# a-lemus96/fs-nerf

Measured on AMD Instinct MI355X. Metric: rendered rays/sec (64+128 samples/ray, 8x256 MLP), higher is better.
Workload: dtype fp16x3

## Files before the change

### fs-nerf_amd/core/models.py

```python
import warnings
from typing import Optional, Sequence, Tuple

import torch
from torch import Tensor, nn
from torch.autograd.function import once_differentiable

from .. import _lib as L
from .. import ops


def _freqs(n_freqs: int, log_space: bool) -> Tensor:
    if log_space:
        return 2.0 ** torch.linspace(0.0, n_freqs - 1, n_freqs)
    return torch.linspace(2.0 ** 0.0, 2.0 ** (n_freqs - 1), n_freqs)


class PositionalEncoder(nn.Module):
    def __init__(self, d_input: int, n_freqs: int, log_space: bool = False):
        super().__init__()
        self.d_input, self.n_freqs, self.log_space = d_input, n_freqs, log_space
        self.d_output = d_input * (1 + 2 * n_freqs)
        self.freqs = [float(f) for f in _freqs(n_freqs, log_space)] if n_freqs > 0 else []

    def forward(self, x: Tensor, mask: Optional[Tensor] = None) -> Tensor:
# ... 155 lines not shown
        self.pos_mask, self.dir_mask = pos_mask, dir_mask

    def train_prec(self) -> int:
        tp = self.train_precision or self.precision
        if tp == "fp16x2":
            tp = "fp16x3"
        return self.PRECISIONS[tp]

    @staticmethod
    def fp16_family(prec: int) -> bool:
        return prec in (L.FSN_PREC_FP16X3, L.FSN_PREC_FP16, L.FSN_PREC_FP16X2)

    @property
    def fp16_mode(self) -> bool:
        return self.fp16_family(self.PRECISIONS[self.precision])

    def _bwd_stage_state(self, dev, which: str = ""):
        st = getattr(self, "_bwd_stage" + which)
        if st is None or st[0].device != dev:
            n = self.n_layers + 2
            st = (torch.ones(n, dtype=torch.float32, device=dev), torch.zeros(n, dtype=torch.int32, device=dev))
            setattr(self, "_bwd_stage" + which, st)
            setattr(self, "_bwd_calibrated" + which, False)
        return st

    def _fold_input_status(self, word: Tensor, dev) -> None:
        w = self._input_word
        if w is None or w.device != dev:
            w = self._input_word = torch.zeros(1, dtype=torch.int32, device=dev)
        w.bitwise_or_(word)
        self._input_calls += 1
        if self.range_check and self._input_calls % self.range_check_every == 0:
            bits = int(w.item())
            if bits:
                w.zero_()
            if bits & L.FSN_STATUS_GRAD_RANGE:
                self.grad_overflow_looks += 1
            if bits & (L.FSN_STATUS_FP16_RANGE | L.FSN_STATUS_FP16_SMALL):
                self.fall_back("input-gradient calls (a flagged call's gradients were written as zeros)", bits, scaled=False)

    def _step_flags(self, dev):
        flags, loose = {}, False
        for p in self.parameters():
            f = getattr(p, "_fsn_step_flag", None)
            if f is None or f.device != dev:
                loose = True
            else:
                flags[id(f)] = f
        out = list(flags.values())
        if loose or not out:
            out.append(ops.step_flag(dev))
        return out

    def _train_status(self, dev) -> Tensor:
        w = self._train_word
        if w is None or w.device != dev:
            w = self._train_word = torch.zeros(2, dtype=torch.int32, device=dev)
        return w

    def fold_status(self, word: Tensor, dev, slot: int) -> None:
        for f in self._step_flags(dev):
            f.bitwise_or_(word)
        self._train_status(dev)[slot:slot + 1].bitwise_or_(word)

    def _read_train_status(self, dev) -> Tuple[int, int]:
        w = self._train_status(dev)
        from ..shard import max_bits_over_ranks
        local, samp = (int(v) for v in w.tolist())
        if local & L.FSN_STATUS_GRAD_RANGE:
            self.grad_overflow_looks += 1
        env = L.FSN_STATUS_FP16_RANGE | L.FSN_STATUS_FP16_SMALL
        bits = max_bits_over_ranks(local & env, dev)
        sbits = max_bits_over_ranks(samp & env, dev)
        if local or samp or bits or sbits:
            w.zero_()
        return bits & env, sbits & env

    def fall_back(self, what: str, bits: int = L.FSN_STATUS_FP16_RANGE, probe=None, earlier_invalid: bool = False,
                  scaled: bool = True) -> None:
        self.range_events += 1
        if scaled and self.infer_prec() == L.FSN_PREC_FP16X3U and self._recalibrate(bits, probe):
            if earlier_invalid:
                warnings.warn(f"fs-nerf HIP path: {what}: the per-layer activation scales did not fit the data "
                              f"({ops.describe_flags(bits)}); re-calibrated", RuntimeWarning, stacklevel=3)
            return
        new = self.FALLBACK.get(self.precision, "bf16x3")
        warnings.warn(f"fs-nerf HIP path: {what}: hidden activations left the fp16 range envelope of precision "
                      f"'{self.precision}' ({ops.describe_flags(bits)}); re-running / continuing in '{new}'",
                      RuntimeWarning, stacklevel=3)
        self.precision = new
        if self.train_precision in self.FALLBACK:
            self.train_precision = None

    def _tensors(self):
        mods = list(self.layers) + [self.sigma, self.connection, self.branch, self.rgb]
        return [m.weight for m in mods], [m.bias for m in mods]

    ACT_TARGET_EXP = 10
    PROBE_MAX = 16384

    def infer_prec(self) -> int:
        if self.precision == "fp16x3" and self.act_scaling:
            return L.FSN_PREC_FP16X3U
        return self.PRECISIONS[self.precision]

    def _param_key(self):
        ws, bs = self._tensors()
        return tuple((t.data_ptr(), t._version) for t in ws + bs)

    def load_state_dict(self, *args, **kwargs):
        out = super().load_state_dict(*args, **kwargs)
        self._act_exps = None
        self._forget_target_moves()
        return out

    def _forget_target_moves(self) -> None:
        self.act_target_exp -= self._target_moved_by
        self._target_moved_by = self._calib_moves = 0

    def _default_probe(self, dev):
        g = torch.Generator(device="cpu").manual_seed(0)
        x = (torch.rand(4096, 3, generator=g) * 4.0 - 2.0).to(dev)
        d = torch.nn.functional.normalize(torch.randn(4096, 3, generator=g), dim=-1).to(dev)
        return x, d

    @torch.no_grad()
    def calibrate(self, probe=None, keep_if_close: bool = False) -> list:
        import math
        ws, bs = self._tensors()
        dev = ws[0].device
        if callable(probe):
            probe = probe()
        x, d = probe if probe is not None else self._default_probe(dev)
        x, d = x.reshape(-1, 3).to(dev, torch.float32), d.reshape(-1, 3).to(dev, torch.float32)
        if x.shape[0] == 0:
            x, d = self._default_probe(dev)
        if x.shape[0] > self.PROBE_MAX:
            idx = torch.linspace(0, x.shape[0] - 1, self.PROBE_MAX, device=dev).long()
            x, d = x[idx], d[idx]
        desc = ops.make_desc(self.n_layers, self.d_hidden, self.skip, self.pos_encoder.freqs, self.dir_encoder.freqs)
        if self._calib_blob is None or self._calib_blob.blob.device != dev:
            self._calib_blob = ops.PackedMLP(desc, L.FSN_PREC_BF16X3, dev)
        self._calib_blob.pack(ws, bs)
        maxima = ops.mlp_layer_maxima(self._calib_blob, x.contiguous(), d.contiguous(), self._mask(self.pos_mask, dev),
                                      self._mask(self.dir_mask, dev))
        D, n = self.d_hidden, self.n_layers
        mods = list(self.layers) + [self.connection, self.branch]
        wmax = []
        for g, m in enumerate(mods):
            w = m.weight.detach().abs()
            na = 0 if g == 0 else D
            wmax.append(w[:, :na].amax() if na else w.new_zeros(()))
            wmax.append(w[:, na:].amax() if w.shape[1] > na else w.new_zeros(()))
        host = torch.cat([maxima, torch.stack(wmax).to(torch.float32)]).cpu().tolist()
        amax, wmx = host[:n + 2], host[n + 2:]
        T = int(self.act_target_exp)
        old = self._act_exps
        exps = []
        for g, v in enumerate(amax):
            if not math.isfinite(v):
                raise RuntimeError(f"NeRF.calibrate: layer {g} produced non-finite activations on the probe batch")
            if v <= 0.0:
                e = old[g] if old is not None else 0
            else:
                e = T - math.ceil(math.log2(v))
                if keep_if_close and old is not None and 2.0 ** (T - 3) <= v * 2.0 ** old[g] <= 2.0 ** (T + 1):
                    e = old[g]
            exps.append(max(-60, min(60, e)))
        for g in range(n + 2):
            prev = 0 if g == 0 else (exps[n - 1] if g == n else (exps[n] if g == n + 1 else exps[g - 1]))
            for wm, sh in ((wmx[2 * g], exps[g] - prev), (wmx[2 * g + 1], exps[g])):
                if wm > 0.0 and math.isfinite(wm):
                    over = math.ceil(math.log2(wm)) + sh - 15
                    if over > 0:
                        exps[g] -= over
        self._act_exps = exps
        self._calib_key = self._param_key()
        self._needs_calibration = False
        self.calibrations += 1
        return exps

    def _recalibrate(self, bits: int, probe) -> bool:
        if self._act_exps is not None and self._calib_key == self._param_key():
            if self._calib_moves >= 3 or bits == (L.FSN_STATUS_FP16_RANGE | L.FSN_STATUS_FP16_SMALL):
                return False
            self._calib_moves += 1
            move = -4 if bits & L.FSN_STATUS_FP16_RANGE else 3
            self.act_target_exp += move
            self._target_moved_by += move
            if not 2 <= self.act_target_exp <= 14:
                return False
        else:
            self._forget_target_moves()
        try:
            self.calibrate(probe)
        except RuntimeError:
            return False
        return True

    def _weights_below_envelope(self) -> bool:
        mods = list(self.layers) + [self.connection, self.branch]
        with torch.no_grad():
            m = torch.stack([mod.weight.detach().abs().amax() for mod in mods])
            return bool(((m > 0) & (m < 2.0 ** -20)).any())

    def _guard_weights(self, what: str, training: bool = False) -> None:
        if not training and self.infer_prec() == L.FSN_PREC_FP16X3U:
            return
        if self.range_check and self.weight_check and self.fp16_mode and self._weights_below_envelope():
            self.fall_back(what + " (a layer's largest weight is below 2^-20)", L.FSN_STATUS_FP16_SMALL, scaled=False)

    def packed(self, probe=None) -> ops.PackedMLP:
        ws, bs = self._tensors()
        scaled = self.infer_prec() == L.FSN_PREC_FP16X3U
        if scaled and (self._act_exps is None or self._needs_calibration):
            self.calibrate(probe, keep_if_close=self._act_exps is not None)
        exps = tuple(self._act_exps) if scaled else None
        key = (self.precision, ws[0].device, exps) + self._param_key()
        if self._packed is None or key != self._packed_key:
            if self._pack_calls % max(1, int(self.range_check_every)) == 0:
                self._guard_weights("NeRF.packed")
                scaled = self.infer_prec() == L.FSN_PREC_FP16X3U
                exps = tuple(self._act_exps) if scaled else None
                key = (self.precision, key[1], exps) + key[3:]
            self._pack_calls += 1
            desc = ops.make_desc(self.n_layers, self.d_hidden, self.skip, self.pos_encoder.freqs,
                                 self.dir_encoder.freqs)
            prec = self.infer_prec()
            if self._packed is None or self._packed.prec != prec or self._packed.blob.device != ws[0].device:
                self._packed = ops.PackedMLP(desc, prec, ws[0].device)
            self._packed.pack(ws, bs, exps)
            self._packed_key = key
        return self._packed

    def packed_single(self, precision: str) -> ops.PackedMLP:
        if precision not in self.SINGLE_PASS:
            raise ValueError(f"single-pass precision: one of {self.SINGLE_PASS}, not {precision!r}")
        ws, bs = self._tensors()
        key = (ws[0].device,) + self._param_key()
        ent = self._packed_single.get(precision)
        if ent is None or ent[0] != key:
            pm = None if ent is None else ent[1]
            if pm is None or pm.blob.device != ws[0].device:
                desc = ops.make_desc(self.n_layers, self.d_hidden, self.skip, self.pos_encoder.freqs, self.dir_encoder.freqs)
                pm = ops.PackedMLP(desc, self.PRECISIONS[precision], ws[0].device)
            pm.pack(ws, bs)
            self._packed_single[precision] = (key, pm)
        return self._packed_single[precision][1]

    def packed_cull(self) -> ops.PackedMLP:
        if self.cull_precision != "bf16":
            raise ValueError("NeRF.cull_precision: None or 'bf16'")
        return self.packed_single(self.cull_precision)

    def occ_eval_fn(self, render_step_size: float, precision: str = "fp16") -> "OccEvalFn":
        return OccEvalFn(self, render_step_size, precision)

    def _autocast_mode(self) -> Optional[str]:
        ap = self.autocast_precision
        if ap is None:
            return None
        if ap not in self.SINGLE_PASS:
            raise ValueError(f"NeRF.autocast_precision: None or one of {self.SINGLE_PASS}, not {ap!r}")
        return ap if not torch.is_grad_enabled() and torch.is_autocast_enabled("cuda") else None

    def _leave_fp16_autocast(self, what: str, bits: int) -> str:
        self.autocast_precision = "bf16"
        return _warn_single_pass(self, what, bits)

    def _mask(self, m: Optional[Tensor], dev) -> Optional[Tensor]:
        return None if m is None else m.to(dev, torch.float32)

    def forward_rays(self, rays_o: Tensor, rays_d: Tensor, ray_indices: Tensor, t_starts: Tensor, t_ends: Tensor,
                     full: bool = True) -> Tensor:
        if full and self._differentiable(rays_o, rays_d):
            ws, bs = self._tensors()
            return _NerfTrainFn.apply(self, (ray_indices, t_starts, t_ends), rays_o, rays_d, *ws, *bs)
        dev = rays_o.device
        args = (rays_o, rays_d, ray_indices, t_starts, t_ends, full, self._mask(self.pos_mask, dev), self._mask(self.dir_mask, dev))

        def probe():
            n = ray_indices.numel()
            idx = torch.linspace(0, max(n - 1, 0), min(n, self.PROBE_MAX), device=dev).long()
            ri = ray_indices[idx].long()
            d = rays_d[ri]
            return rays_o[ri] + d * (t_starts[idx] + t_ends[idx])[:, None] / 2.0, d

        return guarded_launch([self], dev, "NeRF.forward_rays", probe, lambda: ops.mlp_fwd_rays(self.packed(probe), *args))

    def _differentiable(self, *inputs: Optional[Tensor]) -> bool:
        if not torch.is_grad_enabled():
            return False
        if self.training and any(p.requires_grad for p in self.parameters()):
            return True
        return any(t is not None and t.requires_grad for t in inputs)

    def density_gradient(self, x: Tensor) -> Tuple[Tensor, Tensor]:
        xg = x.detach().reshape(-1, 3).to(torch.float32).contiguous().requires_grad_(True)
        dirs = torch.tensor([0.0, 0.0, 1.0], device=xg.device).expand(xg.shape[0], 3).contiguous()
        ws, bs = self._tensors()
        with torch.enable_grad():
            out = _NerfTrainFn.apply(self, None, xg, dirs, *[t.detach() for t in ws + bs])
            cot = torch.zeros_like(out)
            cot[:, 3] = 1.0
            (grad,) = torch.autograd.grad(out, xg, cot)
        return out[:, 3].detach(), grad

    def forward(self, x: Tensor, dirs: Optional[Tensor] = None) -> Tensor:
        if self._differentiable(x, dirs):
            if dirs is None:
                if not self._differentiable():
                    return self._forward_inference(x, dirs)
                raise NotImplementedError(
                    "NeRF.forward(x) with gradients: the density-only pass has no backward (the reference runs it "
                    "under torch.no_grad(), rendering.py:58-64); call it under torch.no_grad() (density_gradient(x) gives "
                    "sigma and its gradient with respect to x)")
            ws, bs = self._tensors()
            return _NerfTrainFn.apply(self, None, x, dirs, *ws, *bs)
        return self._forward_inference(x, dirs)

    def _forward_inference(self, x: Tensor, dirs: Optional[Tensor]) -> Tensor:
        dev = x.device
        mode = self._autocast_mode()
        if mode is not None:
            return single_pass_launch(self, mode, dev, "NeRF.forward (autocast_precision)", self._leave_fp16_autocast,
                                      lambda pm: ops.mlp_fwd(pm, x, dirs, self._mask(self.pos_mask, dev),
                                                             self._mask(self.dir_mask, dev)))

# ... 93 lines not shown
```

### fs-nerf_amd/csrc/host_pack.cpp

```cpp
#include <cstdarg>
#include <cstdio>

#include "mlp_pack.hpp"

static thread_local char g_err[512] = "";
static void set_error(const char* fmt, ...) {
  va_list ap;
  va_start(ap, fmt);
  vsnprintf(g_err, sizeof(g_err), fmt, ap);
  va_end(ap);
}

extern "C" int fsn_version(void) { return 200; }
extern "C" const char* fsn_last_error(void) { return g_err; }

extern "C" int64_t fsn_mlp_blob_bytes(const fsn_mlp_desc* desc, int prec) {
  if (!desc) { set_error("fsn_mlp_blob_bytes: null desc"); return FSN_E_INVALID; }
  fsn::NetGeom G;
  const char* why;
  const int rc = fsn::build_geom(*desc, prec, G, &why);
  if (rc != FSN_OK) { set_error("fsn_mlp_blob_bytes: %s", why); return rc; }
  return G.total_bytes;
}

extern "C" int fsn_mlp_pack_host(const fsn_mlp_desc* desc, int prec, const float* const* weights,
                                 const float* const* biases, void* blob_host) {
  if (!blob_host) { set_error("fsn_mlp_pack_host: null blob"); return FSN_E_INVALID; }
  const char* why;
  const int rc = fsn::pack_blob_host(desc, prec, weights, biases, blob_host, &why);
  if (rc != FSN_OK) set_error("fsn_mlp_pack_host: %s", why);
  return rc;
}

extern "C" int fsn_mlp_pack_scaled_host(const fsn_mlp_desc* desc, int prec, const float* const* weights,
                                        const float* const* biases, const int32_t* layer_exps, void* blob_host) {
  if (!blob_host) { set_error("fsn_mlp_pack_scaled_host: null blob"); return FSN_E_INVALID; }
  const char* why;
  const int rc = fsn::pack_blob_host(desc, prec, weights, biases, blob_host, &why, layer_exps);
  if (rc != FSN_OK) set_error("fsn_mlp_pack_scaled_host: %s", why);
  return rc;
}
```

### fs-nerf_amd/csrc/mlp.hip

```cpp
#include "common.hpp"
#define FSN_X3_PF1
#define FSN_BF16X3_ONEACC 1
#include "mlp_dev.hpp"
#include "mlp_layout.hpp"
#include "mlp_pack.hpp"

#include <cstring>
#include <vector>

namespace fsn {

__global__ void k_pack_stream(PackArgs a, char* __restrict__ blob, int64_t n_pieces) {
  const int64_t piece = (int64_t)blockIdx.x * blockDim.x + threadIdx.x;
  if (piece >= n_pieces) return;
  uint16_t o[8];
  pack_piece(a, piece, o);
  uint4 v;
  v.x = o[0] | ((uint32_t)o[1] << 16);
  v.y = o[2] | ((uint32_t)o[3] << 16);
  v.z = o[4] | ((uint32_t)o[5] << 16);
  v.w = o[6] | ((uint32_t)o[7] << 16);
  *reinterpret_cast<uint4*>(blob + a.G.stream_off + piece * 16) = v;
}

__global__ void k_pack_aux(PackArgs a, char* __restrict__ blob) {
  const int i = blockIdx.x * blockDim.x + threadIdx.x;
  if (i < 64) {
    uint32_t hw[64];
    header_words(a, hw);
    uint32_t w = 0;
#pragma unroll
    for (int k = 0; k < 64; ++k) w = (k == i) ? hw[k] : w;
    reinterpret_cast<uint32_t*>(blob)[i] = w;
  }
  if (i < a.G.aux_floats) reinterpret_cast<float*>(blob + a.G.aux_off)[i] = aux_value(a, i);
}

static int fill_pack_args(const fsn_mlp_desc* d, int prec, const float* const* W, const float* const* b,
                          PackArgs& a, const int32_t* exps = nullptr) {
  const char* why;
  const int rc = fill_pack_args_raw(d, prec, W, b, a, &why, exps);
  FSN_REQUIRE(rc == FSN_OK, rc, "mlp_pack: %s", why);
  return FSN_OK;
}

struct MlpFwdArgs {
  NetParams net;
  const float* x;
  const float* dirs;
  const float* pos_mask;
  const float* dir_mask;
  int64_t n;
  float* out;
  const float *rays_o, *rays_d, *t0, *t1;
  const int64_t* ri;
  int32_t full;
};

template <int NT, int PREC, bool FULL>
__global__ __launch_bounds__(kThreads) void k_mlp_fwd(MlpFwdArgs a) {
  constexpr int NG = groups_per_wave<NT, PREC>(), TILE = 128 * NG;
  __shared__ __attribute__((aligned(1024))) char smem[kRingBytes + (kAuxCapFloats + 96) * 4 + TILE * 6 * 4];
  float* aux_lds = reinterpret_cast<float*>(smem + kRingBytes);
  float* in_lds = aux_lds + kAuxCapFloats + 96;
  NetDev net;
  load_net(a.net, a.pos_mask, a.dir_mask, aux_lds, net);
  __syncthreads();
  constexpr bool full = FULL;
  const int64_t ntiles = (a.n + TILE - 1) / TILE;
  WStream st;
  const char* sbase = a.net.blob + a.net.stream_off;
  st.init(smem, nullptr, 0, 0, sbase, (uint32_t)(full ? a.net.nph_full : a.net.nph_density), 1);
  const int wave = threadIdx.x >> 6, lane = threadIdx.x & 63;
  ARing ring;
  prime_ring<PREC, NT>(st, ring);
  for (int64_t tile = blockIdx.x; tile < ntiles; tile += gridDim.x) {
    if (lane < 16 * NG) {
      const int64_t s = tile * TILE + wave * (16 * NG) + lane;
      const int64_t sc = s < a.n ? s : a.n - 1;
      float* q = in_lds + (wave * (16 * NG) + lane) * 6;
      if (a.ri) {
        ray_sample(a.rays_o, a.rays_d, a.ri, a.t0, a.t1, sc, q, full);
      } else {
        q[0] = a.x[3 * sc]; q[1] = a.x[3 * sc + 1]; q[2] = a.x[3 * sc + 2];
        if (full) { q[3] = a.dirs[3 * sc]; q[4] = a.dirs[3 * sc + 1]; q[5] = a.dirs[3 * sc + 2]; }
      }
    }
    __builtin_amdgcn_wave_barrier();
    const int64_t s0 = tile * TILE + tile_slot<NG>(wave, lane, 0);
    TileSrc src[NG];
    FSN_PER_GROUP(q, src[q] = TileSrc{in_lds + tile_slot<NG>(wave, lane, q) * 6};);
    float sigma[NG], rgb[NG][3] = {};
    mlp_tile<NT, PREC, FULL>(st, net, src, ring, sigma, rgb);
    if (tile_stores<NG>(lane) && s0 + 16 * tile_store_group<NG>(lane) < a.n) {
      const int qs = tile_store_group<NG>(lane);
      const int64_t s = s0 + 16 * qs;
      if (full) {
        f32x4 o = {rgb[qs][0], rgb[qs][1], rgb[qs][2], sigma[qs]};
        *reinterpret_cast<f32x4*>(a.out + 4 * s) = o;
      } else {
        a.out[s] = sigma[qs];
      }
    }
  }
  st.drain();
}

struct MaxSave {
  static constexpr bool kSave = false;
  struct Hook {
    static constexpr bool kZeroInit = false;
    static constexpr bool kPacked = false;
    static constexpr bool kLayerEnd = false;
    float m;
    __device__ __forceinline__ void pre(int) {}
    __device__ __forceinline__ void post(int, float (&v)[8]) {
#pragma unroll
      for (int j = 0; j < 8; ++j) m = fmaxf(m, fabsf(v[j]));
    }
  };
  float* wave_max;
  __device__ __forceinline__ Hook hidden(int) const { return Hook{0.f}; }
  __device__ __forceinline__ Hook branch() const { return Hook{0.f}; }
  __device__ __forceinline__ uint32_t* enc_pos(int) const { return nullptr; }
  __device__ __forceinline__ uint32_t* enc_dir(int) const { return nullptr; }
  __device__ __forceinline__ void layer_done(int l, Hook& hk) const {
    float m = hk.m;
#pragma unroll
    for (int off = 32; off >= 1; off >>= 1) m = fmaxf(m, __shfl_xor(m, off, 64));
    if ((threadIdx.x & 63) == 0) wave_max[l] = fmaxf(wave_max[l], m);
  }
};

template <int NT, int PREC>
__global__ __launch_bounds__(kThreads) void k_mlp_maxima(MlpFwdArgs a, float* __restrict__ maxima) {
  constexpr int TILE = 128, NSLOT = kMaxLayers + 2;
  __shared__ __attribute__((aligned(1024))) char smem[kRingBytes + (kAuxCapFloats + 96) * 4 + TILE * 6 * 4 + kWaves * NSLOT * 4];
  float* aux_lds = reinterpret_cast<float*>(smem + kRingBytes);
  float* in_lds = aux_lds + kAuxCapFloats + 96;
  float* max_lds = in_lds + TILE * 6;
  NetDev net;
  load_net(a.net, a.pos_mask, a.dir_mask, aux_lds, net);
  net.status = nullptr;
  for (int i = threadIdx.x; i < kWaves * NSLOT; i += blockDim.x) max_lds[i] = 0.f;
  __syncthreads();
  const int64_t ntiles = (a.n + TILE - 1) / TILE;
  WStream st;
  st.init(smem, nullptr, 0, 0, a.net.blob + a.net.stream_off, (uint32_t)a.net.nph_full, 1);
  const int wave = threadIdx.x >> 6, lane = threadIdx.x & 63;
  ARing ring;
  prime_ring<PREC, NT>(st, ring);
  const MaxSave sv{max_lds + wave * NSLOT};
  for (int64_t tile = blockIdx.x; tile < ntiles; tile += gridDim.x) {
    if (lane < 16) {
      const int64_t s = tile * TILE + wave * 16 + lane;
      const int64_t sc = s < a.n ? s : a.n - 1;
      float* q = in_lds + (wave * 16 + lane) * 6;
      q[0] = a.x[3 * sc]; q[1] = a.x[3 * sc + 1]; q[2] = a.x[3 * sc + 2];
      q[3] = a.dirs[3 * sc]; q[4] = a.dirs[3 * sc + 1]; q[5] = a.dirs[3 * sc + 2];
    }
    __builtin_amdgcn_wave_barrier();
    const TileSrc src[1] = {{in_lds + tile_slot<1>(wave, lane, 0) * 6}};
    float sigma[1], rgb[1][3] = {};
    mlp_tile<NT, PREC, true>(st, net, src, ring, sigma, rgb, sv);
  }
  st.drain();
  __syncthreads();
  if ((int)threadIdx.x < a.net.n_layers + 2) {
    float m = 0.f;
    for (int w = 0; w < kWaves; ++w) m = fmaxf(m, max_lds[w * NSLOT + threadIdx.x]);
    atomicMax(reinterpret_cast<unsigned int*>(maxima) + threadIdx.x, __float_as_uint(m));
  }
}

template <int NT, int PREC>
static int launch_mlp_maxima(const MlpFwdArgs& a, float* maxima, int cus, hipStream_t s) {
  const int64_t ntiles = (a.n + 127) / 128;
  const unsigned grid = (unsigned)(ntiles < cus ? ntiles : cus);
  k_mlp_maxima<NT, PREC><<<grid, kThreads, 0, s>>>(a, maxima);
  FSN_LAUNCH_CHECK("k_mlp_maxima");
  return FSN_OK;
}

template <int NT, int PREC>
static int launch_mlp_fwd(const MlpFwdArgs& a, int cus, hipStream_t s) {
  constexpr int TILE = 128 * groups_per_wave<NT, PREC>();
  const int64_t ntiles = (a.n + TILE - 1) / TILE;
  const unsigned grid = (unsigned)(ntiles < cus ? ntiles : cus);
  if (a.dirs || (a.ri && a.full)) k_mlp_fwd<NT, PREC, true><<<grid, kThreads, 0, s>>>(a);
  else k_mlp_fwd<NT, PREC, false><<<grid, kThreads, 0, s>>>(a);
  FSN_LAUNCH_CHECK("k_mlp_fwd");
  return FSN_OK;
}

}

using namespace fsn;

extern "C" int64_t fsn_mlp_blob_bytes(const fsn_mlp_desc* desc, int prec) {
  FSN_REQUIRE(desc, FSN_E_INVALID, "fsn_mlp_blob_bytes: null desc");
  NetGeom G;
  const char* why;
  const int rc = build_geom(*desc, prec, G, &why);
  FSN_REQUIRE(rc == FSN_OK, rc, "fsn_mlp_blob_bytes: %s", why);
  return G.total_bytes;
}

extern "C" int fsn_mlp_pack(const fsn_mlp_desc* desc, int prec, const float* const* weights, const float* const* biases,
                            void* blob, fsn_stream_t stream) {
  return fsn_mlp_pack_scaled(desc, prec, weights, biases, nullptr, blob, stream);
}

extern "C" int fsn_mlp_pack_scaled(const fsn_mlp_desc* desc, int prec, const float* const* weights,
                                   const float* const* biases, const int32_t* layer_exps, void* blob, fsn_stream_t stream) {
  FSN_REQUIRE(blob, FSN_E_INVALID, "fsn_mlp_pack: null blob");
  PackArgs a;
  const int rc = fill_pack_args(desc, prec, weights, biases, a, layer_exps);
  if (rc != FSN_OK) return rc;
  const int64_t n_pieces = (int64_t)a.G.nph_full * kPhaseBytes / 16;
  k_pack_stream<<<(unsigned)((n_pieces + 255) / 256), 256, 0, as_stream(stream)>>>(a, static_cast<char*>(blob), n_pieces);
  FSN_LAUNCH_CHECK("k_pack_stream");
  const int naux = a.G.aux_floats > 64 ? a.G.aux_floats : 64;
  k_pack_aux<<<(unsigned)((naux + 255) / 256), 256, 0, as_stream(stream)>>>(a, static_cast<char*>(blob));
  FSN_LAUNCH_CHECK("k_pack_aux");
  return FSN_OK;
}

extern "C" int fsn_mlp_pack_host(const fsn_mlp_desc* desc, int prec, const float* const* weights,
                                 const float* const* biases, void* blob_host) {
  FSN_REQUIRE(blob_host, FSN_E_INVALID, "fsn_mlp_pack_host: null blob");
  const char* why;
  const int rc = pack_blob_host(desc, prec, weights, biases, blob_host, &why);
  FSN_REQUIRE(rc == FSN_OK, rc, "fsn_mlp_pack_host: %s", why);
  return FSN_OK;
}

extern "C" int fsn_mlp_pack_scaled_host(const fsn_mlp_desc* desc, int prec, const float* const* weights,
                                        const float* const* biases, const int32_t* layer_exps, void* blob_host) {
  FSN_REQUIRE(blob_host, FSN_E_INVALID, "fsn_mlp_pack_scaled_host: null blob");
  const char* why;
  const int rc = pack_blob_host(desc, prec, weights, biases, blob_host, &why, layer_exps);
  FSN_REQUIRE(rc == FSN_OK, rc, "fsn_mlp_pack_scaled_host: %s", why);
  return FSN_OK;
}

static int mlp_fwd_any(const char* who, const fsn_mlp_desc* desc, int prec, const void* blob, MlpFwdArgs a, uint32_t* status,
                       fsn_stream_t stream) {
  FSN_REQUIRE(desc && a.n >= 0, FSN_E_INVALID, "%s: bad arguments", who);
  NetGeom G;
  const char* why;
  const int rc = build_geom(*desc, prec, G, &why);
  FSN_REQUIRE(rc == FSN_OK, rc, "%s: %s", who, why);
  if (a.n == 0) return FSN_OK;
  FSN_REQUIRE(blob && a.out && (a.x || (a.ri && a.rays_o && a.rays_d && a.t0 && a.t1)), FSN_E_INVALID, "%s: null pointer", who);
  FSN_REQUIRE(G.aux_floats <= kAuxCapFloats, FSN_E_UNSUPPORTED, "%s: network too deep for the LDS aux area", who);
  const int cus = fsn_device_cus();
  if (cus <= 0) return FSN_E_HIP;
  a.net = net_params(*desc, G, blob, status);
  hipStream_t s = as_stream(stream);
  return dispatch_net(PrecInference{}, desc->d_hidden, prec, [&](auto NT, auto PREC) { return launch_mlp_fwd<NT(), PREC()>(a, cus, s); });
}

extern "C" int fsn_mlp_fwd(const fsn_mlp_desc* desc, int prec, const void* blob, const float* x, const float* dirs,
                           const float* pos_mask, const float* dir_mask, int64_t n, float* out, uint32_t* status,
                           fsn_stream_t stream) {
  MlpFwdArgs a{};
  a.x = x; a.dirs = dirs; a.pos_mask = pos_mask; a.dir_mask = dir_mask; a.n = n; a.out = out;
  return mlp_fwd_any("fsn_mlp_fwd", desc, prec, blob, a, status, stream);
}

extern "C" int fsn_mlp_fwd_rays(const fsn_mlp_desc* desc, int prec, const void* blob, const float* rays_o,
                                const float* rays_d, const int64_t* ray_indices, const float* t_starts,
                                const float* t_ends, int full, const float* pos_mask, const float* dir_mask, int64_t n,
                                float* out, uint32_t* status, fsn_stream_t stream) {
  MlpFwdArgs a{};
  a.rays_o = rays_o; a.rays_d = rays_d; a.ri = ray_indices; a.t0 = t_starts; a.t1 = t_ends; a.full = full ? 1 : 0;
  a.pos_mask = pos_mask; a.dir_mask = dir_mask; a.n = n; a.out = out;
  return mlp_fwd_any("fsn_mlp_fwd_rays", desc, prec, blob, a, status, stream);
}

extern "C" int fsn_mlp_layer_maxima(const fsn_mlp_desc* desc, int prec, const void* blob, const float* x, const float* dirs,
                                    const float* pos_mask, const float* dir_mask, int64_t n, float* maxima,
                                    fsn_stream_t stream) {
  FSN_REQUIRE(desc && n >= 0, FSN_E_INVALID, "fsn_mlp_layer_maxima: bad arguments");
  FSN_REQUIRE(prec == FSN_PREC_BF16X3 || prec == FSN_PREC_FP16X3U, FSN_E_UNSUPPORTED,
              "fsn_mlp_layer_maxima: precision mode %d (FSN_PREC_BF16X3 or FSN_PREC_FP16X3U)", prec);
  NetGeom G;
  const char* why;
  const int rc = build_geom(*desc, prec, G, &why);
  FSN_REQUIRE(rc == FSN_OK, rc, "fsn_mlp_layer_maxima: %s", why);
  if (n == 0) return FSN_OK;
  FSN_REQUIRE(blob && x && dirs && maxima, FSN_E_INVALID, "fsn_mlp_layer_maxima: null pointer");
  FSN_REQUIRE(G.aux_floats <= kAuxCapFloats, FSN_E_UNSUPPORTED, "fsn_mlp_layer_maxima: network too deep for the LDS aux area");
  const int cus = fsn_device_cus();
  if (cus <= 0) return FSN_E_HIP;
  MlpFwdArgs a{};
  a.x = x; a.dirs = dirs; a.pos_mask = pos_mask; a.dir_mask = dir_mask; a.n = n;
  a.net = net_params(*desc, G, blob, nullptr);
  hipStream_t s = as_stream(stream);
  return dispatch_net(PrecModes<FSN_PREC_BF16X3, FSN_PREC_FP16X3U>{}, desc->d_hidden, prec,
                      [&](auto NT, auto PREC) { return launch_mlp_maxima<NT(), PREC()>(a, maxima, cus, s); });
}
```

### fs-nerf_amd/csrc/mlp_dev.hpp

```cpp
#pragma once
#include "common.hpp"
#include "mlp_layout.hpp"
#ifndef FSN_KLOOP_HEADER
#define FSN_KLOOP_HEADER "kloop_gen.hpp"
#endif
#include FSN_KLOOP_HEADER

#include <type_traits>
#include <utility>

namespace fsn {

typedef __attribute__((ext_vector_type(8))) __bf16 bf16x8;
typedef __attribute__((ext_vector_type(8))) _Float16 f16x8;
typedef __attribute__((ext_vector_type(8))) short s16x8;
typedef __attribute__((ext_vector_type(4))) float f32x4;

constexpr int kNSlot = 4;
constexpr int kLead = 2;
constexpr int kLook = 2;
static_assert(kNSlot >= kLook + 2, "ring safety");
constexpr int kLoaders = 4;
constexpr int kLoaderXor = 4;
constexpr int kOpenVmcnt = (kLook - 1) * (kPhaseBytes / 1024 / kLoaders);
static_assert(kOpenVmcnt == 4, "the generated k-loop blocks wait with vmcnt(4)");
__device__ __forceinline__ uint32_t slot_add(uint32_t s, uint32_t k) {
  static_assert((kNSlot & (kNSlot - 1)) == 0, "power-of-two ring");
  return (s + k) & (kNSlot - 1);
}
constexpr int kWaves = 8;
constexpr int kThreads = 64 * kWaves;
constexpr int kGldsPerWave = kPhaseBytes / 1024 / kLoaders;
constexpr int kRingBytes = kNSlot * kPhaseBytes;
constexpr int kAuxCapFloats = 3456;
constexpr int kTileCols = 128;
constexpr int kTRow = 16;
template <int NT, int PREC>
constexpr int groups_per_wave() { return (!prec_is_x3(PREC) && NT == 8) ? 2 : 1; }
template <int NG>
__device__ __forceinline__ constexpr int tile_slot(int wave, int lane, int q) {
  return (wave * NG + q) * 16 + (lane & 15);
}
template <int NG>
__device__ __forceinline__ constexpr bool tile_stores(int lane) { return lane < 16 * NG; }
template <int NG>
__device__ __forceinline__ constexpr int tile_store_group(int lane) {
  static_assert(NG == 1 || NG == 2, "sample groups per wave");
  return (lane >> 4) & (NG - 1);
}
__host__ __device__ constexpr int64_t t_layout_off(int NPL, int P, int pr, int s) {
  return (((int64_t)(s >> 4) * P + pr) * kTRow + (s & 15)) * NPL;
}

#ifndef FSN_BF16X3_ONEACC
#define FSN_BF16X3_ONEACC 0
#endif
constexpr bool prec_one_acc(int P) { return P == FSN_PREC_FP16X3U || (FSN_BF16X3_ONEACC && P == FSN_PREC_BF16X3); }

struct Frag {
  s16x8 hi, lo;
};

struct WStream {
  char* ring;
  uint32_t ring_lds;
  uint32_t m0_base;
  uint32_t is_loader;
  const char *ptrA, *ptrB;
  uint32_t nphA, nphB, repA, repB;
  const char* s_ptr;
  uint32_t s_left, s_which, s_rep, s_slot;
#ifdef FSN_STAMP
  uint64_t t_k = 0, t_e = 0, t_n = 0, t_ko = 0, t_eo = 0;
#endif
  uint32_t c_slot;
  const char* c_base;
  const char* n_base;

  __device__ __forceinline__ void begin_pass_(uint32_t which) {
    s_which = which;
    s_ptr = which ? ptrB : ptrA;
    s_left = which ? nphB : nphA;
  }
  __device__ __forceinline__ void advance_pass_() {
    const uint32_t my_rep = s_which ? repB : repA;
    if (++s_rep >= my_rep) {
      s_rep = 0;
      const uint32_t other = s_which ^ 1u;
      const uint32_t other_rep = other ? repB : repA;
      begin_pass_(other_rep ? other : s_which);
    } else {
      begin_pass_(s_which);
    }
  }
  __device__ __forceinline__ void stage() {
    const uint32_t m0v = m0_base + s_slot * kPhaseBytes;
    const uint32_t voff = ((threadIdx.x >> 6) ^ kLoaderXor) * (kGldsPerWave * 1024) + (threadIdx.x & 63) * 16;
    const uint64_t sbase = (uint64_t)s_ptr;
    uint32_t keep;
    if (is_loader) {
      asm volatile(
          "s_mov_b32 %0, m0\n\t"
          "s_mov_b32 m0, %2\n\t"
          "s_nop 0\n\t"
          "global_load_lds_dwordx4 %1, %3\n\t"
          "global_load_lds_dwordx4 %1, %3 offset:1024\n\t"
          "global_load_lds_dwordx4 %1, %3 offset:2048\n\t"
          "global_load_lds_dwordx4 %1, %3 offset:3072\n\t"
          "s_mov_b32 m0, %0"
          : "=&s"(keep)
          : "v"(voff), "s"(m0v), "s"(sbase)
          : "memory");
    }
    static_assert(kGldsPerWave == 4, "stage() issues exactly 4 loads per loader wave");
    s_ptr += kPhaseBytes;
    s_slot = slot_add(s_slot, 1);
    if (__builtin_expect(--s_left == 0, 0)) {
      asm volatile("" ::: "memory");
      advance_pass_();
    }
  }
  __device__ __forceinline__ void init(char* ring_, const char* pA, uint32_t nA, uint32_t rA, const char* pB,
                                       uint32_t nB, uint32_t rB) {
    ring = ring_;
    ring_lds = (uint32_t)(uintptr_t)(__attribute__((address_space(3))) char*)ring_;
    m0_base = __builtin_amdgcn_readfirstlane(ring_lds + ((threadIdx.x >> 6) ^ kLoaderXor) * (kGldsPerWave * 1024));
    is_loader = __builtin_amdgcn_readfirstlane((((threadIdx.x >> 6) ^ kLoaderXor) < (uint32_t)kLoaders) ? 1u : 0u);
    ptrA = pA; nphA = nA; repA = nA ? rA : 0;
    ptrB = pB; nphB = nB; repB = nB ? rB : 0;
    s_rep = 0; s_slot = 0; c_slot = 0;
    begin_pass_(repA ? 0u : 1u);
    c_base = n_base = ring + (threadIdx.x & 63) * 16;
#pragma unroll
    for (int i = 0; i < kLook; ++i) stage();
    open_next();
  }
  static constexpr uint32_t kDynamicPhases = 1u << 30;
  __device__ __forceinline__ void begin_tile(uint32_t nph) { s_left = nph - (uint32_t)(kLook + 1); }
  __device__ __forceinline__ void open_next() {
    asm volatile("s_waitcnt vmcnt(%0)\n\ts_barrier" ::"n"(kOpenVmcnt) : "memory");
    stage();
    n_base = ring + c_slot * kPhaseBytes + (threadIdx.x & 63) * 16;
    c_slot = slot_add(c_slot, 1);
  }
  __device__ __forceinline__ void enter_phase() { c_base = n_base; }
  __device__ __forceinline__ void next_stage(uint32_t& m0v, uint64_t& gbase) {
    m0v = m0_base + s_slot * kPhaseBytes;
    gbase = (uint64_t)s_ptr;
    s_ptr += kPhaseBytes;
    s_slot = slot_add(s_slot, 1);
    if (__builtin_expect(--s_left == 0, 0)) {
      asm volatile("" ::: "memory");
      advance_pass_();
    }
  }
  __device__ __forceinline__ uint32_t phase_lds(uint32_t k) const {
    return ring_lds + slot_add(slot_add(c_slot, kNSlot - 1), k) * kPhaseBytes + (threadIdx.x & 63) * 16;
  }
  __device__ __forceinline__ void opened(uint32_t n) {
    c_slot = slot_add(c_slot, n);
    n_base = ring + slot_add(c_slot, kNSlot - 1) * kPhaseBytes + (threadIdx.x & 63) * 16;
    c_base = n_base;
  }
  __device__ __forceinline__ void pass_begin() const {}
  __device__ __forceinline__ void pass_end() const {}
  __device__ __forceinline__ void drain() {
    asm volatile("s_waitcnt vmcnt(0) lgkmcnt(0)\n\ts_barrier" ::: "memory");
  }
};

__device__ __forceinline__ void lds_barrier() {
  asm volatile("s_waitcnt lgkmcnt(0)\n\ts_barrier" ::: "memory");
}

template <bool F16>
__device__ __forceinline__ short to_h(float v) {
  if (F16) { const _Float16 h = (_Float16)v; return __builtin_bit_cast(short, h); }
  const __bf16 h = (__bf16)v;
  return __builtin_bit_cast(short, h);
}
template <bool F16>
__device__ __forceinline__ float from_h(short b) {
  if (F16) return (float)__builtin_bit_cast(_Float16, b);
  return (float)__builtin_bit_cast(__bf16, b);
}
template <bool F16, bool X3, bool LS = (F16 && X3)>
__device__ __forceinline__ void split_store_cpp(const float v[8], Frag& f) {
  constexpr float K = LS ? kLoScaleF16 : 1.0f;
#pragma unroll
  for (int j = 0; j < 8; ++j) {
    const short h = to_h<F16>(v[j]);
    f.hi[j] = h;
    f.lo[j] = X3 ? to_h<F16>((v[j] - from_h<F16>(h)) * K) : (short)0;
  }
}

template <bool F16, bool X3, bool LS = (F16 && X3)>
__device__ __forceinline__ void split_store(const float v[8], Frag& f) {
  if constexpr (F16 && X3 && !LS) {
    typedef __attribute__((ext_vector_type(4))) uint32_t u32x4;
    u32x4 h, l;
#pragma unroll
    for (int i = 0; i < 4; ++i) {
      uint32_t hh, ll;
      asm("v_cvt_pk_f16_f32 %0, %2, %3\n\t"
          "v_fma_mixlo_f16 %1, %0, -1.0, %2 op_sel_hi:[1,0,0]\n\t"
          "v_fma_mixhi_f16 %1, %0, -1.0, %3 op_sel:[1,0,0] op_sel_hi:[1,0,0]"
          : "=&v"(hh), "=&v"(ll)
          : "v"(v[2 * i]), "v"(v[2 * i + 1]));
      h[i] = hh;
      l[i] = ll;
    }
    f.hi = __builtin_bit_cast(s16x8, h);
    f.lo = __builtin_bit_cast(s16x8, l);
    return;
  }
  if constexpr (F16 && X3 && LS) {
    typedef __attribute__((ext_vector_type(4))) uint32_t u32x4;
    u32x4 h, l;
    const float kk = kLoScaleF16;
#pragma unroll
    for (int i = 0; i < 4; ++i) {
      uint32_t hh, ll;
      float ra, rb;
      asm("v_cvt_pk_f16_f32 %0, %4, %5\n\t"
          "v_fma_mix_f32 %2, %0, -1.0, %4 op_sel_hi:[1,0,0]\n\t"
          "v_fma_mix_f32 %3, %0, -1.0, %5 op_sel:[1,0,0] op_sel_hi:[1,0,0]\n\t"
          "v_fma_mixlo_f16 %1, %2, %6, 0 op_sel_hi:[0,0,0]\n\t"
          "v_fma_mixhi_f16 %1, %3, %6, 0 op_sel_hi:[0,0,0]"
          : "=&v"(hh), "=&v"(ll), "=&v"(ra), "=&v"(rb)
          : "v"(v[2 * i]), "v"(v[2 * i + 1]), "s"(kk));
      h[i] = hh;
      l[i] = ll;
    }
    f.hi = __builtin_bit_cast(s16x8, h);
    f.lo = __builtin_bit_cast(s16x8, l);
    return;
  }
  split_store_cpp<F16, X3, LS>(v, f);
}

template <bool SIGNED>
__device__ __forceinline__ void range_track(uint32_t& fmax, const s16x8& hi) {
  typedef __attribute__((ext_vector_type(4))) uint32_t u32x4;
  const u32x4 w = __builtin_bit_cast(u32x4, hi);
  if constexpr (!SIGNED) {
    asm("v_pk_maximum3_f16 %0, %0, %1, %2" : "+v"(fmax) : "v"(w[0]), "v"(w[1]));
    asm("v_pk_maximum3_f16 %0, %0, %1, %2" : "+v"(fmax) : "v"(w[2]), "v"(w[3]));
    return;
  }
#pragma unroll
  for (int i = 0; i < 4; ++i) {
    uint32_t x = w[i] & 0x7fff7fffu;
    asm("v_pk_max_u16 %0, %0, %1" : "+v"(fmax) : "v"(x));
  }
}

constexpr uint32_t kSmallBits = 0x0400u;

struct RangeState {
  uint32_t fmax;
  uint32_t fall;
  uint32_t small;
};

constexpr uint32_t kSmallBitsU = 0x2c00u;

template <bool SMALL, uint32_t BITS = kSmallBits>
__device__ __forceinline__ void range_layer_end(RangeState& r) {
  asm("v_pk_max_u16 %0, %0, %1" : "+v"(r.fall) : "v"(r.fmax));
  if constexpr (SMALL) {
    const uint32_t lo = r.fmax & 0xffffu, hi = r.fmax >> 16;
    const uint32_t m = lo > hi ? lo : hi;
    const int any_big = __builtin_amdgcn_readfirstlane((int)__any(m >= BITS));
    const int any_nz = __builtin_amdgcn_readfirstlane((int)__any(m != 0u));
    if (!any_big && any_nz) r.small = 1u;
  }
  r.fmax = 0u;
}

__device__ __forceinline__ void range_report(uint32_t* status, const RangeState& r, uint32_t range_bit = 1u) {
  const uint32_t f = r.fall;
  const bool bad = (f & 0xffffu) >= 0x7c00u || (f >> 16) >= 0x7c00u;
  uint32_t bits = __builtin_amdgcn_readfirstlane((int)__any(bad)) ? range_bit : 0u;
  if (__builtin_amdgcn_readfirstlane((int)r.small)) bits |= 2u;
  if (bits && status) { if ((threadIdx.x & 63) == 0) __hip_atomic_fetch_or(status, bits, __ATOMIC_RELAXED, __HIP_MEMORY_SCOPE_AGENT); }
}

struct NetParams {
  const char* blob;
  int32_t aux_off, aux_floats, stream_off;
  int32_t nph_density, nph_full;
  int32_t n_layers;
  uint32_t skip_mask;
  int32_t n_freqs_pos, n_freqs_dir;
  uint32_t* status;
};

inline NetParams net_params(const fsn_mlp_desc& d, const NetGeom& G, const void* blob, uint32_t* status) {
  NetParams p;
  p.blob = static_cast<const char*>(blob);
  p.aux_off = (int32_t)G.aux_off; p.aux_floats = G.aux_floats; p.stream_off = (int32_t)G.stream_off;
  p.nph_density = G.nph_density; p.nph_full = G.nph_full;
  p.n_layers = d.n_layers; p.skip_mask = d.skip_mask;
  p.n_freqs_pos = d.n_freqs_pos; p.n_freqs_dir = d.n_freqs_dir;
  p.status = status;
  return p;
}

template <int... MODES>
struct PrecModes {};
template <int... MODES, class F>
inline int dispatch_net(PrecModes<MODES...>, int d_hidden, int prec, F&& f) {
  int rc = FSN_E_UNSUPPORTED;
  auto mode = [&](auto PREC) {
    if (prec != decltype(PREC)::value) return false;
    if (d_hidden == 256) rc = f(std::integral_constant<int, 8>{}, PREC);
    else if (d_hidden == 128) rc = f(std::integral_constant<int, 4>{}, PREC);
    return true;
  };
  (void)(mode(std::integral_constant<int, MODES>{}) || ...);
  return rc;
}
template <int... MODES, class F>
inline int dispatch_prec(PrecModes<MODES...>, int prec, F&& f) {
  int rc = FSN_E_UNSUPPORTED;
  auto mode = [&](auto PREC) { return prec == decltype(PREC)::value && (rc = f(PREC), true); };
  (void)(mode(std::integral_constant<int, MODES>{}) || ...);
  return rc;
}
using PrecInference = PrecModes<FSN_PREC_BF16X3, FSN_PREC_BF16, FSN_PREC_FP16X3, FSN_PREC_FP16, FSN_PREC_FP16X3U, FSN_PREC_FP16X2>;
using PrecTraining = PrecModes<FSN_PREC_BF16X3, FSN_PREC_BF16, FSN_PREC_FP16X3, FSN_PREC_FP16>;

struct NetDev {
  const float* aux;
  const float* pos_mask;
  const float* dir_mask;
  int32_t n_layers;
  uint32_t skip_mask;
  int32_t n_freqs_pos, n_freqs_dir;
  uint32_t* status;
};

__device__ __forceinline__ void sincos_f32(float a, float& s_out, float& c_out) {
  const float n = rintf(a * 0.63661977236758134f);
  float r = __builtin_fmaf(-n, 1.57079625129699707031e+00f, a);
  r = __builtin_fmaf(-n, 7.54978941586159635335e-08f, r);
  r = __builtin_fmaf(-n, 5.39030252995776476554e-15f, r);
  const float r2 = r * r;
  float ps = __builtin_fmaf(r2, -1.9515295891e-4f, 8.3321608736e-3f);
  ps = __builtin_fmaf(r2, ps, -1.6666654611e-1f);
  const float sn = __builtin_fmaf(r * r2, ps, r);
  float pc = __builtin_fmaf(r2, 2.443315711809948e-5f, -1.388731625493765e-3f);
  pc = __builtin_fmaf(r2, pc, 4.166664568298827e-2f);
  const float cs = __builtin_fmaf(r2 * r2, pc, __builtin_fmaf(r2, -0.5f, 1.0f));
  const int q = (int)n & 3;
  const float s1 = (q & 1) ? cs : sn;
  const float c1 = (q & 1) ? sn : cs;
  s_out = (q & 2) ? -s1 : s1;
  c_out = ((q + 1) & 2) ? -c1 : c1;
}

template <int NKS, bool F16, bool X3, bool SAVE = false, bool LS = (F16 && X3)>
__device__ __forceinline__ void encode(float x0, float x1, float x2, int n_freqs, const float* __restrict__ freqs,
                                       const float* __restrict__ mask, int g, Frag (&out)[NKS], uint32_t* save = nullptr) {
  constexpr int SLOTS = 8 * NKS;
  float v[SLOTS];
  const int P = 3 * n_freqs;
#pragma unroll
  for (int i = 0; i < SLOTS / 2; ++i) {
    const int p = 4 * i + g;
    const bool ok = p < P;
    const int ps = ok ? p : 0;
    const int band = (ps * 11) >> 5;
    const int coord = ps - 3 * band;
    const float xc = coord == 0 ? x0 : (coord == 1 ? x1 : x2);
    float s, c;
    if constexpr (X3) {
      sincos_f32(xc * freqs[band], s, c);
    } else {
      const float rev = (xc * freqs[band]) * 0.15915494309189535f;
      const float fr = __builtin_amdgcn_fractf(rev);
      s = __builtin_amdgcn_sinf(fr);
      c = __builtin_amdgcn_cosf(fr);
    }
    v[2 * i] = ok ? s * mask[3 + band * 6 + coord] : 0.f;
    v[2 * i + 1] = ok ? c * mask[3 + band * 6 + 3 + coord] : 0.f;
  }
  if (g == 2) {
    v[SLOTS - 2] = x0 * mask[0];
    v[SLOTS - 1] = x1 * mask[1];
  }
  if (g == 3) v[SLOTS - 2] = x2 * mask[2];
#pragma unroll
  for (int k = 0; k < NKS; ++k) split_store<F16, X3, LS>(&v[8 * k], out[k]);
  if constexpr (SAVE) {
    typedef __attribute__((ext_vector_type(4))) uint32_t u32x4;
    typedef __attribute__((ext_vector_type(2))) uint32_t u32x2;
#pragma unroll
    for (int k = 0; k < NKS; ++k) {
      const u32x4 h = __builtin_bit_cast(u32x4, out[k].hi), l = __builtin_bit_cast(u32x4, out[k].lo);
#pragma unroll
      for (int i = 0; i < 4; ++i) {
        if (X3) __builtin_nontemporal_store((u32x2){h[i], l[i]}, reinterpret_cast<u32x2*>(save + (16 * k + i) * kTRow * 2));
        else __builtin_nontemporal_store(h[i], save + (16 * k + i) * kTRow);
      }
    }
  }
}

enum : int { EPI_RELU_CVT = 0, EPI_LAST_FULL = 1, EPI_LAST_DENS = 4, EPI_CVT = 2, EPI_RGB = 3, EPI_NONE = 5 };

struct Heads {
  float sigma;
  float rgb[3];
  RangeState rs;
};

template <bool F16>
__device__ __forceinline__ f32x4 mfma16(const s16x8& a, const s16x8& b, const f32x4& c) {
  if (F16)
    return __builtin_amdgcn_mfma_f32_16x16x32_f16(__builtin_bit_cast(f16x8, a), __builtin_bit_cast(f16x8, b), c, 0, 0, 0);
  return __builtin_amdgcn_mfma_f32_16x16x32_bf16(__builtin_bit_cast(bf16x8, a), __builtin_bit_cast(bf16x8, b), c, 0, 0, 0);
}
struct AFrag {
  s16x8 hi, lo;
};
constexpr int kKD = FSN_KLOOP_D;
constexpr int kNS = FSN_KLOOP_NSETS;
struct ARing {
  AFrag cur[kNS > 3 ? kNS : 3];
};
template <int PREC>
__device__ __forceinline__ void load_afrag(const char* p, AFrag& f) {
  f.hi = *reinterpret_cast<const s16x8*>(p);
  if (prec_reads_w_lo(PREC)) f.lo = *reinterpret_cast<const s16x8*>(p + 1024);
}
template <int PREC>
__device__ __forceinline__ void unit_mfma_r(const AFrag& a, const Frag& b, f32x4& acc, f32x4& cor) {
  constexpr bool F16 = prec_is_f16(PREC), X3 = prec_is_x3(PREC);
  acc = mfma16<F16>(a.hi, b.hi, acc);
  if (X3) {
    f32x4& c = prec_one_acc(PREC) ? acc : cor;
    if (prec_reads_w_lo(PREC)) c = mfma16<F16>(a.lo, b.hi, c);
    c = mfma16<F16>(a.hi, b.lo, c);
  }
}

template <int PREC>
__device__ __forceinline__ void unit_mfma(const char* ubase, const Frag& b, f32x4& acc, f32x4& cor) {
  constexpr bool F16 = prec_is_f16(PREC), X3 = prec_is_x3(PREC);
  const s16x8 ah = *reinterpret_cast<const s16x8*>(ubase);
  acc = mfma16<F16>(ah, b.hi, acc);
  if (X3) {
    f32x4& c = prec_one_acc(PREC) ? acc : cor;
    if (prec_reads_w_lo(PREC)) {
      const s16x8 al = *reinterpret_cast<const s16x8*>(ubase + 1024);
      c = mfma16<F16>(al, b.hi, c);
// ... 358 lines not shown

template <int PREC, int NP_OUT, int KS_ACT, int KS_ENC, int EPI, int NACT, int NENC, int NOUT>
__device__ __forceinline__ void gemm_layer_two_groups(WStream& st, const NetDev& net, int aux_bias,
                                                      const Frag (&act)[2][NACT], const Frag (&enc)[2][NENC],
                                                      Frag (&out)[2][NOUT], Heads (&heads)[2], ARing& ring, int g) {
  constexpr bool F16 = prec_is_f16(PREC);
  static_assert(!prec_is_x3(PREC), "two groups per wave: single-pass modes only");
  constexpr int UPP = 16, UB = 1024;
  constexpr int KS = KS_ACT + KS_ENC;
  constexpr int TOTAL = 2 * NP_OUT * KS;
  static_assert(KS_ACT <= NACT && KS_ENC <= NENC, "operand arrays too small");
  const float* bias = net.aux + aux_bias;
  NoHook hk;
#pragma unroll
  for (int tp = 0; tp < NP_OUT; ++tp) {
    const f32x4 b0 = *reinterpret_cast<const f32x4*>(bias + 32 * tp + 4 * g);
    const f32x4 b1 = *reinterpret_cast<const f32x4*>(bias + 32 * tp + 16 + 4 * g);
    f32x4 a00 = b0, a01 = b1, a10 = b0, a11 = b1;
#pragma unroll
    for (int ks = 0; ks < KS; ++ks) {
      const Frag& x0 = ks < KS_ACT ? act[0][ks < KS_ACT ? ks : 0] : enc[0][ks >= KS_ACT ? ks - KS_ACT : 0];
      const Frag& x1 = ks < KS_ACT ? act[1][ks < KS_ACT ? ks : 0] : enc[1][ks >= KS_ACT ? ks - KS_ACT : 0];
      const int u = (tp * KS + ks) * 2;
      if (((u + kLead) % UPP == 0 && u + kLead <= TOTAL) || (u + kLead == TOTAL && TOTAL % UPP != 0)) st.open_next();
      if (u % UPP == 0) st.enter_phase();
      AFrag nxt[2];
      const int v = u + 2;
      const char* src = (v < TOTAL) ? ((v / UPP == u / UPP) ? st.c_base : st.n_base) + (v % UPP) * UB
                                    : st.n_base + (v - TOTAL) * UB;
      load_afrag<PREC>(src, nxt[0]);
      load_afrag<PREC>(src + UB, nxt[1]);
      a00 = mfma16<F16>(ring.cur[0].hi, x0.hi, a00);
      a10 = mfma16<F16>(ring.cur[0].hi, x1.hi, a10);
      a01 = mfma16<F16>(ring.cur[1].hi, x0.hi, a01);
      a11 = mfma16<F16>(ring.cur[1].hi, x1.hi, a11);
      ring.cur[0] = nxt[0];
      ring.cur[1] = nxt[1];
      __builtin_amdgcn_sched_group_barrier(0x100, 2, 0);
      __builtin_amdgcn_sched_group_barrier(0x008, 4, 0);
      __builtin_amdgcn_sched_barrier(0);
    }
    pair_epilogue<PREC, NP_OUT, EPI>(net, tp, a00, a01, a00, a01, out[0], heads[0], g, hk);
    pair_epilogue<PREC, NP_OUT, EPI>(net, tp, a10, a11, a10, a11, out[1], heads[1], g, hk);
  }
}

template <int PREC, int NT = 0>
__device__ __forceinline__ void prime_ring(const WStream& st, ARing& ring) {
  constexpr int UB = prec_is_x3(PREC) ? 2048 : 1024;
  if (kKloopAsm && prec_is_x3(PREC) && NT == 8) {
#pragma unroll
    for (int i = 0; i < kKD; ++i) load_afrag<PREC>(st.n_base + i * UB, ring.cur[i]);
#pragma unroll
    for (int i = kKD; i < (kNS > 3 ? kNS : 3); ++i) ring.cur[i] = ring.cur[0];
    return;
  }
#ifdef FSN_X3_PF1
  if (prec_is_x3(PREC)) {
    load_afrag<PREC>(st.n_base, ring.cur[0]);
    return;
  }
#else
  if (prec_is_x3(PREC)) return;
#endif
  load_afrag<PREC>(st.n_base, ring.cur[0]);
  load_afrag<PREC>(st.n_base + UB, ring.cur[1]);
  if (!prec_is_x3(PREC)) ring.cur[0].lo = ring.cur[1].lo = ring.cur[0].hi;
}

struct NoSave {
  static constexpr bool kSave = false;
  using Hook = NoHook;
  __device__ __forceinline__ Hook hidden(int) const { return {}; }
  __device__ __forceinline__ Hook branch() const { return {}; }
  __device__ __forceinline__ uint32_t* enc_pos(int) const { return nullptr; }
  __device__ __forceinline__ uint32_t* enc_dir(int) const { return nullptr; }
  __device__ __forceinline__ void layer_done(int, Hook&) const {}
};

#define FSN_PER_GROUP(Q, ...)               \
  do {                                      \
    {                                       \
      constexpr int Q = 0;                  \
      __VA_ARGS__                           \
    }                                       \
    if constexpr (NG == 2) {                \
      constexpr int Q = NG - 1;             \
      __VA_ARGS__                           \
    }                                       \
  } while (0)

#define FSN_TEMPLATE_ARGS(...) __VA_ARGS__
#define FSN_GEMM_LAYER(TA, BIAS, IN, ENC, OUT)                                                                          \
  do {                                                                                                                  \
    if constexpr (NG == 1) gemm_layer<FSN_TEMPLATE_ARGS TA>(st, net, BIAS, IN[0], ENC[0], OUT[0], heads[0], ring, g, hk); \
    else gemm_layer_two_groups<FSN_TEMPLATE_ARGS TA>(st, net, BIAS, IN, ENC, OUT, heads, ring, g);                       \
  } while (0)

template <int NT, int PREC, bool FULL, int NG, class Src, class SV>
__device__ __forceinline__ void mlp_tile(WStream& st, const NetDev& net, const Src (&src)[NG], ARing& ring,
                                         float (&sigma)[NG], float (&rgb)[NG][3], const SV& sv) {
  constexpr int NA = NT;
  constexpr bool F16 = prec_is_f16(PREC), X3 = prec_is_x3(PREC), LS = prec_lo_scaled(PREC);
  static_assert(NG == 1 || (NG == 2 && !X3 && std::is_same<SV, NoSave>::value), "sample groups per wave");
  const int g = (threadIdx.x >> 4) & 3;
  constexpr int D = 32 * NT;
  const int L = net.n_layers;
  const float* misc = net.aux + (L + 5) * D;
  Frag A[NG][NA], B[NG][NA];
  Frag none[NG][1];
  Heads heads[NG];
  FSN_PER_GROUP(q, heads[q] = Heads{0.f, {0.f, 0.f, 0.f}, {0u, 0u, 0u}};);
#define FSN_ENC_POS(SAVE, PE)                                                                                 \
  FSN_PER_GROUP(q, float px, py, pz; src[q].pos(px, py, pz);                                                     \
                encode<kKsPos, F16, X3, SAVE, LS>(px, py, pz, net.n_freqs_pos, misc + 4, net.pos_mask, g, PE[q], \
                                                  SAVE ? sv.enc_pos(g) : nullptr);)
  {
    Frag pe[NG][kKsPos];
    FSN_ENC_POS(SV::kSave, pe);
    typename SV::Hook hk = sv.hidden(0);
    FSN_GEMM_LAYER((PREC, NT, 0, kKsPos, EPI_RELU_CVT), 0, none, pe, A);
    sv.layer_done(0, hk);
  }
#define FSN_HIDDEN(EPI, IN, OUT, LIDX)                                                              \
  do {                                                                                              \
    typename SV::Hook hk = sv.hidden(LIDX);                                                         \
    if ((net.skip_mask >> ((LIDX)-1)) & 1u) {                                                       \
      Frag pe2[NG][kKsPos];                                                                         \
      FSN_ENC_POS(false, pe2);                                                                      \
      FSN_GEMM_LAYER((PREC, NT, NA, kKsPos, EPI), (LIDX)*D, IN, pe2, OUT);   \
    } else                                                                                          \
      FSN_GEMM_LAYER((PREC, NT, NA, 0, EPI), (LIDX)*D, IN, none, OUT);       \
    sv.layer_done(LIDX, hk);                                                                        \
  } while (0)
  for (int l = 1; l <= L - 2; l += 2) {
    FSN_HIDDEN(EPI_RELU_CVT, A, B, l);
    if (l + 1 <= L - 2) {
      FSN_HIDDEN(EPI_RELU_CVT, B, A, l + 1);
    } else {
      FSN_PER_GROUP(q, Frag(&a)[NA] = A[q]; const Frag(&b)[NA] = B[q];
                    _Pragma("unroll") for (int i = 0; i < NA; ++i) a[i] = b[i];);
    }
  }
  FSN_HIDDEN((FULL ? EPI_LAST_FULL : EPI_LAST_DENS), A, B, L - 1);
#undef FSN_HIDDEN
#undef FSN_ENC_POS
  {
    float sg[NG];
    FSN_PER_GROUP(q, sg[q] = heads[q].sigma;);
    FSN_PER_GROUP(q, sg[q] += __shfl_xor(sg[q], 16, 64););
    FSN_PER_GROUP(q, sg[q] += __shfl_xor(sg[q], 32, 64););
    FSN_PER_GROUP(q, sigma[q] = sg[q] + misc[0];);
  }
  if (FULL) {
    {
      typename SV::Hook hk = sv.hidden(L);
      FSN_GEMM_LAYER((PREC, NT, NA, 0, EPI_CVT), L * D, B, none, A);
      sv.layer_done(L, hk);
    }
    Frag de[NG][kKsDir];
    FSN_PER_GROUP(q, float dx, dy, dz; src[q].dir(dx, dy, dz);
                  encode<kKsDir, F16, X3, SV::kSave, LS>(dx, dy, dz, net.n_freqs_dir, misc + 20, net.dir_mask, g, de[q], sv.enc_dir(g)););
    {
      typename SV::Hook hk = sv.branch();
      FSN_GEMM_LAYER((PREC, NT / 2, NA, kKsDir, EPI_RGB), (L + 1) * D, A, de, B);
      sv.layer_done(L + 1, hk);
    }
#pragma unroll
    for (int c = 0; c < 3; ++c) {
      float z[NG];
      FSN_PER_GROUP(q, z[q] = heads[q].rgb[c];);
      FSN_PER_GROUP(q, z[q] += __shfl_xor(z[q], 16, 64););
      FSN_PER_GROUP(q, z[q] += __shfl_xor(z[q], 32, 64););
      FSN_PER_GROUP(q, z[q] += misc[1 + c]; rgb[q][c] = 1.0f / (1.0f + expf(-z[q])););
    }
  }
  if constexpr (F16) {
    if constexpr (NG == 2) asm("v_pk_max_u16 %0, %0, %1" : "+v"(heads[0].rs.fmax) : "v"(heads[1].rs.fmax));
    range_layer_end<false>(heads[0].rs);
    range_report(net.status, heads[0].rs);
  }
}

#undef FSN_GEMM_LAYER
#undef FSN_TEMPLATE_ARGS

template <int NT, int PREC, bool FULL, int NG, class Src>
__device__ __forceinline__ void mlp_tile(WStream& st, const NetDev& net, const Src (&src)[NG], ARing& ring,
                                         float (&sigma)[NG], float (&rgb)[NG][3]) {
  mlp_tile<NT, PREC, FULL>(st, net, src, ring, sigma, rgb, NoSave{});
}

struct TileSrc {
  const float* p;
  __device__ __forceinline__ void pos(float& x, float& y, float& z) const { x = p[0]; y = p[1]; z = p[2]; }
  __device__ __forceinline__ void dir(float& x, float& y, float& z) const { x = p[3]; y = p[4]; z = p[5]; }
};

__device__ __forceinline__ void ray_sample(const float* __restrict__ ro, const float* __restrict__ rd,
                                           const int64_t* __restrict__ ri, const float* __restrict__ t0,
                                           const float* __restrict__ t1, int64_t s, float* q, bool with_dir) {
  const int64_t r = ri[s];
  const float tm = t0[s] + t1[s];
#pragma unroll
  for (int c = 0; c < 3; ++c) {
    const float dc = rd[3 * r + c];
    q[c] = ro[3 * r + c] + dc * tm / 2.0f;
    if (with_dir) q[3 + c] = dc;
  }
}

__device__ __forceinline__ void load_net(const NetParams& p, const float* __restrict__ pos_mask_g,
                                         const float* __restrict__ dir_mask_g, float* lds, NetDev& net) {
  const f32x4* src = reinterpret_cast<const f32x4*>(p.blob + p.aux_off);
  f32x4* dst = reinterpret_cast<f32x4*>(lds);
  for (int i = threadIdx.x; i < p.aux_floats / 4; i += blockDim.x) dst[i] = src[i];
  float* pm = lds + p.aux_floats;
  float* dm = pm + 64;
  const int npe = 3 * (1 + 2 * p.n_freqs_pos), nde = 3 * (1 + 2 * p.n_freqs_dir);
  for (int i = threadIdx.x; i < 64; i += blockDim.x) pm[i] = (pos_mask_g && i < npe) ? pos_mask_g[i] : 1.0f;
  for (int i = threadIdx.x; i < 32; i += blockDim.x) dm[i] = (dir_mask_g && i < nde) ? dir_mask_g[i] : 1.0f;
  net.aux = lds;
  net.pos_mask = pm;
  net.dir_mask = dm;
  net.n_layers = p.n_layers;
  net.skip_mask = p.skip_mask;
  net.n_freqs_pos = p.n_freqs_pos;
  net.n_freqs_dir = p.n_freqs_dir;
  net.status = p.status;
}

}
```

### fs-nerf_amd/csrc/mlp_layout.hpp

```cpp
#pragma once
#include <cstdint>

#include "fsnerf_hip.h"

#if defined(__HIPCC__)
#define FSN_HD __host__ __device__ __forceinline__
#else
#define FSN_HD inline
#endif

namespace fsn {

constexpr uint32_t kBlobMagic = 0x4e53460au;
constexpr int kPhaseBytes = 16384;
constexpr int kKsPos = 2;
constexpr int kKsDir = 1;
constexpr int kMaxLayers = 16;

constexpr int kPrecSinglePassBit = 1;
FSN_HD constexpr bool prec_is_x3(int prec) { return (prec & kPrecSinglePassBit) == 0; }
FSN_HD constexpr bool prec_is_f16(int prec) { return prec >= FSN_PREC_FP16X3; }
FSN_HD constexpr bool prec_reads_w_lo(int prec) { return prec_is_x3(prec) && prec != FSN_PREC_FP16X2; }
constexpr float kLoScaleF16 = 2048.0f;
FSN_HD constexpr bool prec_lo_scaled(int prec) { return prec == FSN_PREC_FP16X3 || prec == FSN_PREC_FP16X2; }
FSN_HD float lo_scale(int prec) { return prec_lo_scaled(prec) ? kLoScaleF16 : 1.0f; }
FSN_HD int unit_bytes(int prec) { return prec_is_x3(prec) ? 2048 : 1024; }
FSN_HD int units_per_phase(int prec) { return kPhaseBytes / unit_bytes(prec); }

struct LayerGeom {
  int32_t nt_out;
  int32_t ks_act;
  int32_t ks_enc;
  int32_t enc_is_dir;
  int32_t n_freqs;
  int32_t d_act;
  int32_t ld;
  int32_t unit0;
};

struct NetGeom {
  int32_t n_gemm;
  LayerGeom g[kMaxLayers + 2];
  int32_t units_hidden;
  int32_t units_total;
  int32_t nph_density, nph_full;
  int32_t aux_bias[kMaxLayers + 2];
  int32_t aux_wsigma, aux_wrgb, aux_misc, aux_floats;
  int64_t aux_off, stream_off, total_bytes;
};

FSN_HD int enc_slot_feature(int q, int g, int n_freqs, int slots) {
  const int P = 3 * n_freqs;
  const int np = P > g ? (P - g + 3) / 4 : 0;
  if (q < 2 * np) {
    const int p = 4 * (q >> 1) + g;
    const int band = p / 3, coord = p - 3 * band;
    return 3 + band * 6 + (q & 1) * 3 + coord;
  }
  if (g == 2 && q >= slots - 2) return q - (slots - 2);
  if (g == 3 && q == slots - 2) return 2;
  return -1;
}

FSN_HD int unit_src_col(const LayerGeom& L, int ks, int g, int j) {
  if (ks < L.ks_act) return 32 * ks + 16 * (j >> 2) + 4 * g + (j & 3);
  const int e = ks - L.ks_act;
  const int slots = 8 * L.ks_enc;
  const int f = enc_slot_feature(8 * e + j, g, L.n_freqs, slots);
  return f < 0 ? -1 : L.d_act + f;
}

FSN_HD uint16_t bf16_rne(float f) {
  union { float f; uint32_t u; } v;
  v.f = f;
  if ((v.u & 0x7fffffffu) > 0x7f800000u) return (uint16_t)((v.u >> 16) | 0x40);
  return (uint16_t)((v.u + 0x7fffu + ((v.u >> 16) & 1u)) >> 16);
}
FSN_HD float bf16_to_f32(uint16_t b) {
  union { float f; uint32_t u; } v;
  v.u = (uint32_t)b << 16;
  return v.f;
}

FSN_HD uint16_t f16_rne(float f) {
  union { float f; uint32_t u; } v;
  v.f = f;
  const uint32_t sign = (v.u >> 16) & 0x8000u;
  uint32_t x = v.u & 0x7fffffffu;
  if (x > 0x7f800000u) return (uint16_t)(sign | 0x7e00u);
  if (x >= 0x477ff000u) return (uint16_t)(sign | 0x7c00u);
  if (x < 0x38800000u) {
    v.u = x;
    const float a = v.f * 16777216.0f;
    float r = (float)(int)a;
    const float frac = a - r;
    if (frac > 0.5f || (frac == 0.5f && ((int)r & 1))) r += 1.0f;
    return (uint16_t)(sign | (uint32_t)(int)r);
  }
  x += 0xfffu + ((x >> 13) & 1u);
  return (uint16_t)(sign | ((x - 0x38000000u) >> 13));
}
FSN_HD float f16_to_f32(uint16_t h) {
  union { float f; uint32_t u; } v;
  const uint32_t sign = ((uint32_t)h & 0x8000u) << 16;
  const uint32_t e = (h >> 10) & 31u, m = h & 0x3ffu;
  if (e == 0) {
    v.f = (float)m * 5.9604644775390625e-08f;
    v.u |= sign;
    return v.f;
  }
  v.u = sign | (e == 31 ? 0x7f800000u | (m << 13) : ((e + 112u) << 23) | (m << 13));
  return v.f;
}
FSN_HD uint16_t half_rne(float f, bool f16) { return f16 ? f16_rne(f) : bf16_rne(f); }
FSN_HD float half_to_f32(uint16_t h, bool f16) { return f16 ? f16_to_f32(h) : bf16_to_f32(h); }

inline int build_geom(const fsn_mlp_desc& d, int prec, NetGeom& G, const char** why) {
  *why = "";
  if (prec < 0 || (prec > FSN_PREC_FP16X3U && prec != FSN_PREC_FP16X2)) { *why = "unknown precision mode"; return FSN_E_INVALID; }
  if (d.d_hidden != 256 && d.d_hidden != 128) { *why = "d_hidden must be 128 or 256"; return FSN_E_UNSUPPORTED; }
  if (d.n_layers < 2 || d.n_layers > kMaxLayers) { *why = "n_layers must be in [2,16]"; return FSN_E_UNSUPPORTED; }
  if (d.n_freqs_pos < 0 || d.n_freqs_pos > 10) { *why = "n_freqs (position) must be <= 10"; return FSN_E_UNSUPPORTED; }
  if (d.n_freqs_dir < 0 || d.n_freqs_dir > 4) { *why = "n_freqs (direction) must be <= 4"; return FSN_E_UNSUPPORTED; }
  if (d.skip_mask >> (d.n_layers - 1)) { *why = "skip index >= n_layers-1 (the reference model cannot run it either)"; return FSN_E_INVALID; }
  const int D = d.d_hidden, NT = D / 32, L = d.n_layers;
  const int d_pe = 3 * (1 + 2 * d.n_freqs_pos), d_de = 3 * (1 + 2 * d.n_freqs_dir);
  int u = 0;
  for (int l = 0; l < L; ++l) {
    LayerGeom& g = G.g[l];
    const bool wide = l > 0 && ((d.skip_mask >> (l - 1)) & 1u);
    g.nt_out = NT;
    g.ks_act = l == 0 ? 0 : NT;
    g.ks_enc = (l == 0 || wide) ? kKsPos : 0;
    g.enc_is_dir = 0;
    g.n_freqs = d.n_freqs_pos;
    g.d_act = l == 0 ? 0 : D;
    g.ld = g.d_act + (g.ks_enc ? d_pe : 0);
    g.unit0 = u;
    u += 2 * g.nt_out * (g.ks_act + g.ks_enc);
  }
  G.units_hidden = u;
  LayerGeom& c = G.g[L];
  c = LayerGeom{NT, NT, 0, 0, 0, D, D, u};
  u += 2 * NT * NT;
  LayerGeom& b = G.g[L + 1];
  b = LayerGeom{NT / 2, NT, kKsDir, 1, d.n_freqs_dir, D, D + d_de, u};
  u += 2 * (NT / 2) * (NT + kKsDir);
  G.n_gemm = L + 2;
  G.units_total = u;
  const int upp = units_per_phase(prec);
  if (G.units_hidden % upp) { *why = "internal: hidden units not phase aligned"; return FSN_E_UNSUPPORTED; }
  G.nph_density = G.units_hidden / upp;
  G.nph_full = (G.units_total + upp - 1) / upp;
  int a = 0;
  for (int l = 0; l < L + 2; ++l) { G.aux_bias[l] = a; a += D; }
  G.aux_wsigma = a; a += D;
  G.aux_wrgb = a; a += 2 * D;
  G.aux_misc = a; a += 4 + 32;
  G.aux_floats = (a + 63) / 64 * 64;
  G.aux_off = 256;
  G.stream_off = (G.aux_off + (int64_t)G.aux_floats * 4 + 4095) / 4096 * 4096;
  G.total_bytes = G.stream_off + (int64_t)G.nph_full * kPhaseBytes;
  return FSN_OK;
}

}
```

### fs-nerf_amd/csrc/mlp_pack.hpp

```cpp
#pragma once
#include "mlp_layout.hpp"

namespace fsn {

struct PackArgs {
  NetGeom G;
  const float* W[kMaxLayers + 4];
  const float* b[kMaxLayers + 4];
  int32_t n_layers, d_hidden, prec;
  uint32_t skip_mask;
  int32_t n_freqs_pos, n_freqs_dir;
  float freqs_pos[16], freqs_dir[16];
  int32_t exps[kMaxLayers + 2];
  float sc_act[kMaxLayers + 2], sc_enc[kMaxLayers + 2], sc_bias[kMaxLayers + 2], sc_sigma, sc_rgb;
};

FSN_HD float pow2f(int e) {
  union { float f; uint32_t u; } v;
  v.u = (uint32_t)(e + 127) << 23;
  return v.f;
}

inline void fill_scales(PackArgs& a, const int32_t* exps) {
  const int L = a.n_layers;
  for (int g = 0; g < L + 2; ++g) a.exps[g] = exps ? exps[g] : 0;
  for (int g = L + 2; g < kMaxLayers + 2; ++g) a.exps[g] = 0;
  for (int g = 0; g < L + 2; ++g) {
    const int prev = g == 0 ? 0 : (g <= L ? a.exps[g == L ? L - 1 : g - 1] : a.exps[L]);
    a.sc_act[g] = pow2f(a.exps[g] - prev);
    a.sc_enc[g] = pow2f(a.exps[g]);
    a.sc_bias[g] = pow2f(a.exps[g]);
  }
  a.sc_sigma = pow2f(-a.exps[L - 1]);
  a.sc_rgb = pow2f(-a.exps[L + 1]);
}

FSN_HD int gemm_to_sd(int g, int L) { return g < L ? g : g + 1; }

FSN_HD void pack_piece(const PackArgs& a, int64_t piece, uint16_t out8[8]) {
  const int ub = unit_bytes(a.prec);
  const int ppu = ub / 16;
  const int unit = (int)(piece / ppu);
  const int rem = (int)(piece - (int64_t)unit * ppu);
  const int part = rem >> 6, lane = rem & 63;
  for (int j = 0; j < 8; ++j) out8[j] = 0;
  if (unit >= a.G.units_total) return;
  int g = 0;
  while (g + 1 < a.G.n_gemm && a.G.g[g + 1].unit0 <= unit) ++g;
  const LayerGeom& Lg = a.G.g[g];
  const int ks_tot = Lg.ks_act + Lg.ks_enc;
  const int lu = unit - Lg.unit0;
  const int sub = lu & 1;
  const int t = (lu >> 1) / ks_tot, ks = (lu >> 1) - t * ks_tot;
  const int r = lane & 15, grp = lane >> 4;
  const float* W = a.W[gemm_to_sd(g, a.n_layers)];
  const int row = 32 * t + 16 * sub + r;
  for (int j = 0; j < 8; ++j) {
    const int col = unit_src_col(Lg, ks, grp, j);
    if (col < 0) continue;
    const float w = W[(int64_t)row * Lg.ld + col] * (ks < Lg.ks_act ? a.sc_act[g] : a.sc_enc[g]);
    const bool f16 = prec_is_f16(a.prec);
    const uint16_t hi = half_rne(w, f16);
    out8[j] = part == 0 ? hi : half_rne((w - half_to_f32(hi, f16)) * lo_scale(a.prec), f16);
  }
}

FSN_HD float aux_value(const PackArgs& a, int i) {
  const int D = a.d_hidden, L = a.n_layers;
  const int blk = i / D, off = i - blk * D;
  if (blk < L) return a.b[blk][off] * a.sc_bias[blk];
  if (blk == L) return a.b[L + 1][off] * a.sc_bias[L];
  if (blk == L + 1) return off < D / 2 ? a.b[L + 2][off] * a.sc_bias[L + 1] : 0.f;
  if (blk == L + 2) return a.W[L][off] * a.sc_sigma;
  if (blk == L + 3 || blk == L + 4) {
    const int k = i - (L + 3) * D;
    return k < 3 * (D / 2) ? a.W[L + 3][k] * a.sc_rgb : 0.f;
  }
  const int m = i - (L + 5) * D;
  if (m == 0) return a.b[L][0];
  if (m >= 1 && m <= 3) return a.b[L + 3][m - 1];
  if (m >= 4 && m < 20) return a.freqs_pos[m - 4];
  if (m >= 20 && m < 36) return a.freqs_dir[m - 20];
  return 0.f;
}

FSN_HD void header_words(const PackArgs& a, uint32_t hw[64]) {
  for (int i = 0; i < 64; ++i) hw[i] = 0;
  hw[0] = kBlobMagic; hw[1] = 3;
  for (int g = 0; g < a.n_layers + 2; ++g) hw[16 + g] = (uint32_t)a.exps[g];
  hw[2] = (uint32_t)a.prec; hw[3] = (uint32_t)a.n_layers;
  hw[4] = (uint32_t)a.d_hidden; hw[5] = a.skip_mask; hw[6] = (uint32_t)a.n_freqs_pos;
  hw[7] = (uint32_t)a.n_freqs_dir; hw[8] = (uint32_t)a.G.units_total; hw[9] = (uint32_t)a.G.nph_full;
  hw[10] = (uint32_t)a.G.nph_density; hw[11] = (uint32_t)a.G.aux_off; hw[12] = (uint32_t)a.G.aux_floats;
  hw[13] = (uint32_t)a.G.stream_off; hw[14] = (uint32_t)(a.G.total_bytes & 0xffffffffu);
}


inline int fill_pack_args_raw(const fsn_mlp_desc* d, int prec, const float* const* W, const float* const* b, PackArgs& a,
                              const char** why, const int32_t* exps = nullptr) {
  *why = "";
  if (!d || !W || !b) { *why = "null pointer"; return FSN_E_INVALID; }
  const int rc = build_geom(*d, prec, a.G, why);
  if (rc != FSN_OK) return rc;
  for (int i = 0; i < d->n_layers + 4; ++i) {
    if (!W[i] || !b[i]) { *why = "null weight / bias pointer"; return FSN_E_INVALID; }
    a.W[i] = W[i];
    a.b[i] = b[i];
  }
  a.n_layers = d->n_layers; a.d_hidden = d->d_hidden; a.prec = prec; a.skip_mask = d->skip_mask;
  a.n_freqs_pos = d->n_freqs_pos; a.n_freqs_dir = d->n_freqs_dir;
  for (int i = 0; i < 16; ++i) { a.freqs_pos[i] = d->freqs_pos[i]; a.freqs_dir[i] = d->freqs_dir[i]; }
  if (exps)
    for (int g = 0; g < d->n_layers + 2; ++g)
      if (exps[g] < -60 || exps[g] > 60) { *why = "layer exponent outside [-60, 60]"; return FSN_E_INVALID; }
  fill_scales(a, exps);
  return FSN_OK;
}

inline int pack_blob_host(const fsn_mlp_desc* d, int prec, const float* const* W, const float* const* b, void* blob_host,
                          const char** why, const int32_t* exps = nullptr) {
  PackArgs a;
  const int rc = fill_pack_args_raw(d, prec, W, b, a, why, exps);
  if (rc != FSN_OK) return rc;
  char* blob = static_cast<char*>(blob_host);
  for (int64_t i = 0; i < a.G.total_bytes; ++i) blob[i] = 0;
  uint32_t hw[64];
  header_words(a, hw);
  for (int i = 0; i < 64; ++i) reinterpret_cast<uint32_t*>(blob)[i] = hw[i];
  float* aux = reinterpret_cast<float*>(blob + a.G.aux_off);
  for (int i = 0; i < a.G.aux_floats; ++i) aux[i] = aux_value(a, i);
  const int64_t n_pieces = (int64_t)a.G.nph_full * kPhaseBytes / 16;
  uint16_t* sp = reinterpret_cast<uint16_t*>(blob + a.G.stream_off);
  for (int64_t p = 0; p < n_pieces; ++p) pack_piece(a, p, sp + p * 8);
  return FSN_OK;
}

}
```

### fs-nerf_amd/csrc/render.hip

```cpp
#include "common.hpp"
#define FSN_KLOOP_ASM
#define FSN_BF16X3_ONEACC 1
#include "mlp_dev.hpp"
#include "ray_dev.hpp"

namespace fsn {

FSN_DEBUG_DEFINE_RECORD(g_dbg_render)
#define FSN_DEBUG_RECORD g_dbg_render

constexpr int kMaxGroupSamples = 768;
constexpr int kMaxGroupCoarse = 768;
constexpr int kMaxG = 4;
constexpr int kMaxRaySamples = 384;
struct RenderKArgs {
  NetParams netC, netF;
  fsn_render_args a;
  int32_t G, nsubC, nsubF;
  float step;
  int32_t two_phase;
  float cam_hw, cam_hh, cam_f;
};

struct RenderLds {
  fsn_render_args args;
  int32_t Gc, nsubC, nsubF;
  float step;
  int32_t two_phase;
  float cam_hw, cam_hh, cam_f;
  float rays[kMaxG * 6];
  float edgesC[kMaxGroupCoarse + kMaxG];
  float sigC[kMaxGroupCoarse];
  float wC[kMaxGroupCoarse];
  float edgesF[kMaxGroupSamples + kMaxG];
  float sigF[kMaxGroupSamples];
  float rgbF[3 * kMaxGroupSamples];
  float cdf[kMaxG][kMaxRaySamples + 1];
  float vals[kMaxG][kMaxRaySamples + 1];
};

constexpr int kNetLdsBytes = (kAuxCapFloats + 96) * 4;
constexpr int kRenderLdsBytes = kRingBytes + 2 * kNetLdsBytes + (int)sizeof(RenderLds);
static_assert(kRenderLdsBytes <= 160 * 1024, "LDS budget");

struct RaySrc {
  const float* ray;
  const float* e;
  __device__ __forceinline__ void pos(float& x, float& y, float& z) const {
    const float tm = e[0] + e[1];
    x = ray[0] + ray[3] * tm / 2.0f;
    y = ray[1] + ray[4] * tm / 2.0f;
    z = ray[2] + ray[5] * tm / 2.0f;
  }
  __device__ __forceinline__ void dir(float& x, float& y, float& z) const { x = ray[3]; y = ray[4]; z = ray[5]; }
};

#define GRP_S (a.S)
#define GRP_NI (a.n_imp)
#define GRP_SO (a.S + a.n_imp)
#define GRP_HIER (a.n_imp > 0)
#define GRP_G (S_.Gc)
#define GRP_R (a.R)
#ifdef FSN_STAMP
__device__ unsigned long long g_stamp[256 * 8 * 8];
#endif
template <int NT, int PREC, bool TWO_PHASE>
__global__ __launch_bounds__(kThreads) void k_render_fused(RenderKArgs k) {
#ifdef FSN_STAMP
  const uint64_t t_begin = __builtin_amdgcn_s_memtime();
#endif
  uint64_t clk_t0 = 0, clk_r0 = 0;
  const bool clk_on = k.a.clock_out != nullptr && blockIdx.x == 0 && __builtin_amdgcn_readfirstlane(threadIdx.x) < 64;
  if (clk_on) { clk_t0 = __builtin_amdgcn_s_memtime(); clk_r0 = __builtin_amdgcn_s_memrealtime(); }
  auto clk_end = [&]() __attribute__((always_inline)) {
    if (clk_on && (threadIdx.x & 63) == 0) {
      k.a.clock_out[0] += __builtin_amdgcn_s_memtime() - clk_t0;
      k.a.clock_out[1] += __builtin_amdgcn_s_memrealtime() - clk_r0;
    }
  };
  __shared__ __attribute__((aligned(1024))) char smem[kRenderLdsBytes];
  float* auxC = reinterpret_cast<float*>(smem + kRingBytes);
  float* auxF = reinterpret_cast<float*>(smem + kRingBytes + kNetLdsBytes);
  RenderLds& S_ = *reinterpret_cast<RenderLds*>(smem + kRingBytes + 2 * kNetLdsBytes);
  if (threadIdx.x == 0) S_.args = k.a;
  __syncthreads();
  const fsn_render_args& a = S_.args;
  if (threadIdx.x == 0) {
    S_.Gc = k.G; S_.nsubC = k.nsubC; S_.nsubF = k.nsubF; S_.step = k.step; S_.two_phase = k.two_phase;
    S_.cam_hw = k.cam_hw; S_.cam_hh = k.cam_hh; S_.cam_f = k.cam_f;
  }
  __syncthreads();
  NetDev netC, netF;
  load_net(k.netF, a.pos_mask, a.dir_mask, auxF, netF);
  if (GRP_HIER) load_net(k.netC, a.pos_mask, a.dir_mask, auxC, netC);
  else netC = netF;
  __syncthreads();
  WStream st;
  {
    const int64_t ngr = (k.a.R + k.G - 1) / k.G;
    const int64_t mine = ngr > (int64_t)blockIdx.x ? (ngr - blockIdx.x + gridDim.x - 1) / gridDim.x : 0;
    const uint32_t repC = k.two_phase ? (uint32_t)(mine * k.nsubC) : (uint32_t)k.nsubC;
    const uint32_t repF = k.two_phase == 2 ? 0u : (k.two_phase ? (uint32_t)(mine * k.nsubF) : (uint32_t)k.nsubF);
    st.init(smem, k.netC.blob + k.netC.stream_off, GRP_HIER ? (uint32_t)k.netC.nph_density : 0u, repC,
            k.netF.blob + k.netF.stream_off, (uint32_t)k.netF.nph_full, repF);
  }
  int tid = threadIdx.x, wave = tid >> 6, lane = tid & 63;
#define FSN_RELAUNDER()                                              \
  do {                                                               \
    int t_ = threadIdx.x;                                            \
    asm volatile("" : "+v"(t_));                                     \
    tid = t_; wave = __builtin_amdgcn_readfirstlane(t_ >> 6); lane = t_ & 63; \
  } while (0)
  constexpr int NG = groups_per_wave<NT, PREC>(), TILE = 128 * NG;
  ARing ring;
  prime_ring<PREC, NT>(st, ring);
  auto small_div = [](int n, int d) __attribute__((always_inline)) {
    int q = (int)(((float)n + 0.5f) * __builtin_amdgcn_rcpf((float)d));
    q += (q + 1) * d <= n ? 1 : 0;
    q -= q * d > n ? 1 : 0;
    return q;
  };
  auto load_rays = [&](int64_t r0) __attribute__((always_inline)) {
    if (a.rays_o) {
      if (tid < GRP_G * 6) {
        const int g = tid / 6, c = tid - 6 * g;
        const int64_t ray = min(r0 + g, GRP_R - 1);
        FSN_AT(S_.rays, tid) = c < 3 ? a.rays_o[3 * ray + c] : a.rays_d[3 * ray + c - 3];
      }
    } else if (tid < GRP_G) {
      const int64_t ray = min(r0 + tid, GRP_R - 1);
      const uint32_t Wc = (uint32_t)__builtin_amdgcn_readfirstlane(a.cam_W), rr = (uint32_t)ray;
      const int h = a.cam_row0 + (int)(rr / Wc), w = (int)(rr % Wc);
      float o[3], d[3];
      pinhole_ray(a.cam_pose, S_.cam_hw, S_.cam_hh, S_.cam_f, h, w, o, d);
#pragma unroll
      for (int c = 0; c < 3; ++c) { FSN_AT(S_.rays, 6 * tid + c) = o[c]; FSN_AT(S_.rays, 6 * tid + 3 + c) = d[c]; }
    }
  };
  auto coarse_stage = [&](int64_t r0) __attribute__((always_inline)) {
    for (int e = tid; e < GRP_G * (GRP_S + 1); e += kThreads) {
      const int g = small_div(e, GRP_S + 1), i = e - g * (GRP_S + 1);
      const int64_t ray = min(r0 + g, GRP_R - 1);
      const float* ur = a.u_mode == 1 ? a.u + ray : (a.u_mode == 2 ? a.u + ray * (GRP_S + 1) : nullptr);
      FSN_AT(S_.edgesC, e) = stratified_edge(a.near, S_.step, GRP_S, i, a.u_mode, ur);
    }
    lds_barrier();
    if (!GRP_HIER) return;
    st.pass_begin();
    for (int sub = 0; sub < S_.nsubC; ++sub) {
      auto slot = [&](int q) { return sub * TILE + tile_slot<NG>(wave, lane, q); };
      auto source = [&](int idx) {
        const int idc = min(idx, GRP_G * GRP_S - 1);
        const int g = small_div(idc, GRP_S), i = idc - g * GRP_S;
        return RaySrc{FSN_SPAN(S_.rays, 6 * g, 6), FSN_SPAN(S_.edgesC, g * (GRP_S + 1) + i, 2)};
      };
      const int idx0 = slot(0);
      RaySrc src[NG];
      FSN_PER_GROUP(q, src[q] = source(idx0 + 16 * q););
      float sigma[NG], rgb[NG][3];
      mlp_tile<NT, PREC, false>(st, netC, src, ring, sigma, rgb);
      if (tile_stores<NG>(lane)) {
        const int qs = tile_store_group<NG>(lane), idx = idx0 + 16 * qs;
        if (idx < GRP_G * GRP_S) FSN_AT(S_.sigC, idx) = sigma[qs];
      }
    }
    st.pass_end();
    lds_barrier();
    for (int g = wave; g < GRP_G; g += kWaves) {
      const int64_t ray = min(r0 + g, GRP_R - 1);
      float* wc = FSN_SPAN(S_.wC, g * GRP_S, GRP_S);
      weights_ray(FSN_SPAN(S_.sigC, g * GRP_S, GRP_S), FSN_SPAN(S_.edgesC, g * (GRP_S + 1), GRP_S + 1), GRP_S, wc);
      __builtin_amdgcn_wave_barrier();
      if (a.weights_coarse && r0 + g < GRP_R)
        for (int i = lane; i < GRP_S; i += 64) a.weights_coarse[ray * GRP_S + i] = wc[i];
      sample_pdf_merge_ray(FSN_SPAN(S_.edgesC, g * (GRP_S + 1), GRP_S + 1), wc, GRP_S, GRP_NI,
                           a.u_fine ? a.u_fine + ray * GRP_NI : nullptr, FSN_AT(S_.cdf, g), FSN_AT(S_.vals, g),
                           FSN_SPAN(S_.edgesF, g * (GRP_SO + 1), GRP_SO + 1));
    }
    lds_barrier();
  };
  auto fine_stage = [&](int64_t r0, const float* edges, bool write_edges) __attribute__((always_inline)) {
    st.pass_begin();
    for (int sub = 0; sub < S_.nsubF; ++sub) {
      auto slot = [&](int q) { return sub * TILE + tile_slot<NG>(wave, lane, q); };
      auto source = [&](int idx) {
        const int idc = min(idx, GRP_G * GRP_SO - 1);
        const int g = small_div(idc, GRP_SO), i = idc - g * GRP_SO;
        return RaySrc{FSN_SPAN(S_.rays, 6 * g, 6), edges + g * (GRP_SO + 1) + i};
      };
      const int idx0 = slot(0);
      RaySrc src[NG];
      FSN_PER_GROUP(q, src[q] = source(idx0 + 16 * q););
      float sigma[NG], rgb[NG][3];
      mlp_tile<NT, PREC, true>(st, netF, src, ring, sigma, rgb);
      if (tile_stores<NG>(lane)) {
        const int qs = tile_store_group<NG>(lane), idx = idx0 + 16 * qs;
        if (idx < GRP_G * GRP_SO) {
          FSN_AT(S_.sigF, idx) = sigma[qs];
          FSN_AT(S_.rgbF, 3 * idx + 0) = rgb[qs][0];
          FSN_AT(S_.rgbF, 3 * idx + 1) = rgb[qs][1];
          FSN_AT(S_.rgbF, 3 * idx + 2) = rgb[qs][2];
        }
      }
    }
    st.pass_end();
    lds_barrier();
    for (int g = wave; g < GRP_G; g += kWaves) {
      if (r0 + g >= GRP_R) continue;
      const int64_t ray = r0 + g;
      const float* eg = edges + g * (GRP_SO + 1);
      CompositeOut o{a.colors + 3 * ray, a.opacity + ray, a.depth + ray,
                     a.weights ? a.weights + ray * GRP_SO : nullptr, a.alphas ? a.alphas + ray * GRP_SO : nullptr,
                     a.trans ? a.trans + ray * GRP_SO : nullptr};
      composite_ray(FSN_SPAN(S_.sigF, g * GRP_SO, GRP_SO), FSN_SPAN(S_.rgbF, 3 * g * GRP_SO, 3 * GRP_SO), eg, eg + 1, GRP_SO,
                    true, a.bkgd[0], a.bkgd[1], a.bkgd[2], o);
      if (a.sigmas)
        for (int i = lane; i < GRP_SO; i += 64) a.sigmas[ray * GRP_SO + i] = FSN_AT(S_.sigF, g * GRP_SO + i);
      if (a.rgbs)
        for (int i = lane; i < 3 * GRP_SO; i += 64) a.rgbs[ray * GRP_SO * 3 + i] = FSN_AT(S_.rgbF, 3 * g * GRP_SO + i);
      if (write_edges && a.edges_out)
        for (int i = lane; i <= GRP_SO; i += 64) a.edges_out[ray * (GRP_SO + 1) + i] = eg[i];
    }
    lds_barrier();
  };
  const int64_t ngroups = (GRP_R + GRP_G - 1) / GRP_G;
  if constexpr (!TWO_PHASE) {
    for (int64_t grp = blockIdx.x; grp < ngroups; grp += gridDim.x) {
      FSN_RELAUNDER();
      const int64_t r0 = grp * (int64_t)__builtin_amdgcn_readfirstlane(GRP_G);
      load_rays(r0);
      coarse_stage(r0);
      fine_stage(r0, GRP_HIER ? FSN_SPAN(S_.edgesF, 0, GRP_G * (GRP_SO + 1)) : FSN_SPAN(S_.edgesC, 0, GRP_G * (GRP_SO + 1)), true);
    }
  } else {
    for (int64_t grp = blockIdx.x; grp < ngroups; grp += gridDim.x) {
      FSN_RELAUNDER();
      const int64_t r0 = grp * (int64_t)__builtin_amdgcn_readfirstlane(GRP_G);
      load_rays(r0);
      coarse_stage(r0);
      for (int e = tid; e < GRP_G * (GRP_SO + 1); e += kThreads) {
        const int g = small_div(e, GRP_SO + 1), i = e - g * (GRP_SO + 1);
        if (r0 + g < GRP_R) __builtin_nontemporal_store(FSN_AT(S_.edgesF, e), a.edges_out + (r0 + g) * (GRP_SO + 1) + i);
      }
      lds_barrier();
    }
    __builtin_amdgcn_fence(__ATOMIC_RELEASE, "workgroup");
// ... 1 lines not shown
    __builtin_amdgcn_fence(__ATOMIC_ACQUIRE, "workgroup");
    if (S_.two_phase == 2) {
      st.drain();
      clk_end();
      return;
    }
    for (int64_t grp = blockIdx.x; grp < ngroups; grp += gridDim.x) {
      FSN_RELAUNDER();
      const int64_t r0 = grp * (int64_t)__builtin_amdgcn_readfirstlane(GRP_G);
      load_rays(r0);
      for (int e = tid; e < GRP_G * (GRP_SO + 1); e += kThreads) {
        const int g = small_div(e, GRP_SO + 1), i = e - g * (GRP_SO + 1);
        FSN_AT(S_.edgesF, e) = __builtin_nontemporal_load(a.edges_out + min(r0 + g, GRP_R - 1) * (GRP_SO + 1) + i);
      }
      lds_barrier();
      fine_stage(r0, FSN_SPAN(S_.edgesF, 0, GRP_G * (GRP_SO + 1)), false);
    }
  }
  st.drain();
  clk_end();
#ifdef FSN_STAMP
  if ((threadIdx.x & 63) == 0 && blockIdx.x < 256) {
    unsigned long long* o = g_stamp + (blockIdx.x * 8 + (threadIdx.x >> 6)) * 8;
    o[0] = __builtin_amdgcn_s_memtime() - t_begin; o[1] = st.t_k; o[2] = st.t_e; o[3] = st.t_n;
    o[4] = st.t_ko; o[5] = st.t_eo;
  }
#endif
}

template <int PREC>
__global__ __launch_bounds__(kThreads) void k_bare_stream(const char* stream, uint32_t nph, int layers, uint64_t* clk) {
  __shared__ __attribute__((aligned(1024))) char smem[kRingBytes + 256 * 4];
  float* zeros = reinterpret_cast<float*>(smem + kRingBytes);
  for (int i = threadIdx.x; i < 256; i += blockDim.x) zeros[i] = 0.f;
  __syncthreads();
  NetDev net{};
  net.aux = zeros;
  net.n_layers = 8;
  WStream st;
  st.init(smem, nullptr, 0, 0, stream, nph, 1);
  ARing ring;
  prime_ring<PREC, 8>(st, ring);
  const int g = (threadIdx.x >> 4) & 3;
  Frag A[8], B[8];
  Frag none[1];
  uint32_t h = 0x9e3779b9u * (threadIdx.x + 1u) + 0x85ebca6bu * (blockIdx.x + 1u);
  auto next = [&]() { h ^= h << 13; h ^= h >> 17; h ^= h << 5; return h; };
#pragma unroll
  for (int k = 0; k < 8; ++k)
#pragma unroll
    for (int j = 0; j < 8; ++j) {
      const uint32_t r = next();
      const uint16_t hi = (r & 1u) ? (uint16_t)(0x3c00u + ((r >> 1) % 9u) * 0x0400u + ((r >> 8) & 0x3ffu)) : (uint16_t)0;
      const uint16_t lo = (r & 1u) ? (uint16_t)((hi - 0x2c00u) ^ ((r >> 20) & 0x8000u)) : (uint16_t)0;
      A[k].hi[j] = (short)hi;
      A[k].lo[j] = (short)lo;
    }
  Heads heads{0.f, {0.f, 0.f, 0.f}, {0u, 0u, 0u}};
  const uint64_t t0 = __builtin_amdgcn_s_memtime(), r0 = __builtin_amdgcn_s_memrealtime();
  for (int l = 0; l < layers; ++l) {
    gemm_layer<PREC, 8, 8, 0, EPI_RELU_CVT>(st, net, 0, A, none, B, heads, ring, g);
    asm volatile("" ::"v"(B[0].hi), "v"(B[7].lo));
  }
  const uint64_t t1 = __builtin_amdgcn_s_memtime(), r1 = __builtin_amdgcn_s_memrealtime();
  st.drain();
  if (clk && (threadIdx.x & 63) == 0) {
    uint64_t* o = clk + 2 * (blockIdx.x * kWaves + (threadIdx.x >> 6));
    o[0] = t1 - t0;
    o[1] = r1 - r0;
  }
  if (heads.rs.fall == 0xffffffffu && clk) clk[0] = 0;
}

#undef GRP_S
#undef GRP_NI
#undef GRP_SO
#undef GRP_HIER
#undef GRP_G
#undef GRP_R

template <int NT, int PREC>
static int launch_render(RenderKArgs k, int cus, hipStream_t s) {
  constexpr int kTilesG1 = 2;
  constexpr int NG = groups_per_wave<NT, PREC>(), TILE = 128 * NG, CAP = NG == 1 ? 384 * kTilesG1 : kMaxGroupSamples;
  const int So = k.a.S + k.a.n_imp;
  int g = (NG == 1 ? kTilesG1 : 1) * TILE / k.a.S;
  if (g < 1) g = 1;
  if (g > CAP / So) g = CAP / So;
  if (g > kMaxG) g = kMaxG;
  if (g > kMaxGroupCoarse / k.a.S) g = kMaxGroupCoarse / k.a.S;
  if (g < 1) g = 1;
  k.G = g;
  k.nsubC = (g * k.a.S + TILE - 1) / TILE;
  k.nsubF = (g * So + TILE - 1) / TILE;
  const int64_t ngroups = (k.a.R + k.G - 1) / k.G;
  const unsigned grid = (unsigned)(ngroups < cus ? ngroups : cus);
  if (k.two_phase) k_render_fused<NT, PREC, true><<<grid, kThreads, 0, s>>>(k);
  else k_render_fused<NT, PREC, false><<<grid, kThreads, 0, s>>>(k);
  FSN_LAUNCH_CHECK("k_render_fused");
  return FSN_OK;
}

}

using namespace fsn;

#ifdef FSN_STAMP
extern "C" int fsn_dbg_stamps(unsigned long long* host_out) {
  FSN_HIP(hipDeviceSynchronize());
  FSN_HIP(hipMemcpyFromSymbol(host_out, HIP_SYMBOL(g_stamp), sizeof(unsigned long long) * 256 * 8 * 8));
  return FSN_OK;
}
#endif

extern "C" int fsn_render_rays_fused(const fsn_mlp_desc* desc, int prec, const void* blob_coarse,
                                     const void* blob_fine, const fsn_render_args* args, fsn_stream_t stream) {
  FSN_REQUIRE(desc && args, FSN_E_INVALID, "fsn_render_rays_fused: null pointer");
  const fsn_render_args& a = *args;
  FSN_REQUIRE(a.R >= 0 && a.S > 0 && a.n_imp >= 0 && a.u_mode >= 0 && a.u_mode <= 2, FSN_E_INVALID,
              "fsn_render_rays_fused: bad sizes R=%lld S=%d n_imp=%d u_mode=%d", (long long)a.R, a.S, a.n_imp, a.u_mode);
  NetGeom G;
  const char* why;
  const int rc = build_geom(*desc, prec, G, &why);
  FSN_REQUIRE(rc == FSN_OK, rc, "fsn_render_rays_fused: %s", why);
  if (a.R == 0) return FSN_OK;
  const bool sampler_only = a.two_phase == 2;
  if (sampler_only) {
    FSN_REQUIRE(a.n_imp > 0 && blob_coarse && a.edges_out, FSN_E_INVALID,
                "fsn_render_rays_fused: two_phase == 2 (sampler only) needs n_imp > 0, blob_coarse and edges_out");
    if (!blob_fine) blob_fine = blob_coarse;
  } else {
    FSN_REQUIRE(blob_fine && a.colors && a.opacity && a.depth, FSN_E_INVALID, "fsn_render_rays_fused: null pointer");
  }
  if (a.rays_o) {
    FSN_REQUIRE(a.rays_d, FSN_E_INVALID, "fsn_render_rays_fused: rays_o without rays_d");
  } else {
    FSN_REQUIRE(a.cam_H > 0 && a.cam_W > 0 && a.cam_focal > 0 && a.cam_row0 >= 0 &&
                    (int64_t)a.cam_H * a.cam_W < (1ll << 31) && a.R <= (int64_t)(a.cam_H - a.cam_row0) * a.cam_W,
                FSN_E_INVALID, "fsn_render_rays_fused: no rays and no valid camera (H=%d W=%d focal=%g row0=%d R=%lld)",
                a.cam_H, a.cam_W, a.cam_focal, a.cam_row0, (long long)a.R);
  }
  FSN_REQUIRE(a.n_imp == 0 || blob_coarse, FSN_E_INVALID, "fsn_render_rays_fused: hierarchical sampling needs blob_coarse");
  FSN_REQUIRE(a.u_mode == 0 || a.u, FSN_E_INVALID, "fsn_render_rays_fused: u_mode %d needs u", a.u_mode);
  const int So = a.S + a.n_imp;
  FSN_REQUIRE(So <= kMaxRaySamples, FSN_E_UNSUPPORTED, "fsn_render_rays_fused: S+n_imp=%d > %d", So, kMaxRaySamples);
  {
    int n2 = 1;
    while (n2 < a.n_imp) n2 <<= 1;
    FSN_REQUIRE(a.S + n2 <= kMaxRaySamples, FSN_E_UNSUPPORTED, "fsn_render_rays_fused: S + pow2ceil(n_imp) = %d > %d",
                a.S + n2, kMaxRaySamples);
  }
  FSN_REQUIRE(G.aux_floats <= kAuxCapFloats, FSN_E_UNSUPPORTED, "fsn_render_rays_fused: network too deep for LDS");
  RenderKArgs k;
  k.netF = net_params(*desc, G, blob_fine, a.status);
  k.netC = net_params(*desc, G, a.n_imp > 0 ? blob_coarse : blob_fine, a.status);
  k.a = a;
  k.G = k.nsubC = k.nsubF = 0;
  k.step = (float)(((double)a.far - (double)a.near) / a.S);
  k.two_phase = sampler_only ? 2 : ((a.two_phase && a.n_imp > 0 && a.edges_out) ? 1 : 0);
  k.cam_hw = (float)(a.cam_W * 0.5);
  k.cam_hh = (float)(a.cam_H * 0.5);
  k.cam_f = (float)a.cam_focal;
  const int cus = fsn_device_cus();
  if (cus <= 0) return FSN_E_HIP;
  hipStream_t s = as_stream(stream);
  return dispatch_net(PrecInference{}, desc->d_hidden, prec, [&](auto NT, auto PREC) { return launch_render<NT(), PREC()>(k, cus, s); });
}

extern "C" int fsn_bench_bare_stream(const fsn_mlp_desc* desc, int prec, const void* blob, int layers, uint64_t* clock_out,
                                     fsn_stream_t stream) {
  FSN_REQUIRE(desc && blob && layers > 0, FSN_E_INVALID, "fsn_bench_bare_stream: bad arguments");
  FSN_REQUIRE(desc->d_hidden == 256 && (prec == FSN_PREC_BF16X3 || prec == FSN_PREC_FP16X3 || prec == FSN_PREC_FP16X3U),
              FSN_E_UNSUPPORTED, "fsn_bench_bare_stream: d_hidden 256 in an x3 mode only");
  NetGeom G;
  const char* why;
  const int rc = build_geom(*desc, prec, G, &why);
  FSN_REQUIRE(rc == FSN_OK, rc, "fsn_bench_bare_stream: %s", why);
  const int cus = fsn_device_cus();
  if (cus <= 0) return FSN_E_HIP;
  const char* sp = static_cast<const char*>(blob) + G.stream_off;
  hipStream_t s = as_stream(stream);
  const int launched = dispatch_prec(PrecModes<FSN_PREC_BF16X3, FSN_PREC_FP16X3, FSN_PREC_FP16X3U>{}, prec, [&](auto PREC) {
    k_bare_stream<PREC()><<<cus, kThreads, 0, s>>>(sp, (uint32_t)G.nph_density, layers, clock_out);
    FSN_LAUNCH_CHECK("k_bare_stream");
    return FSN_OK;
  });
  return launched == FSN_OK ? cus : launched;
}

namespace fsn { int debug_report_occ(unsigned* host4); }

#ifdef FSN_DEBUG
namespace fsn {
__global__ void k_debug_selftest(int n) {
  __shared__ float arr[32];
  arr[threadIdx.x & 31] = 0.f;
  __syncthreads();
  if (threadIdx.x == 0) {
    FSN_AT(arr, n) = 1.f;
    float* p = FSN_SPAN(arr, 30, 4);
    p[0] = 2.f;
  }
}
}
#endif

extern "C" int fsn_debug_selftest(void) {
#ifdef FSN_DEBUG
  fsn::k_debug_selftest<<<1, 64>>>(32);
  FSN_LAUNCH_CHECK("k_debug_selftest");
  return FSN_OK;
#else
  FSN_REQUIRE(false, FSN_E_UNSUPPORTED, "fsn_debug_selftest: not a debug build");
#endif
}

extern "C" int fsn_debug_report(uint32_t* out_host) {
  FSN_REQUIRE(out_host, FSN_E_INVALID, "fsn_debug_report: null pointer");
#ifdef FSN_DEBUG
  FSN_HIP(hipDeviceSynchronize());
  unsigned zero[4] = {0u, 0u, 0u, 0u};
  FSN_HIP(hipMemcpyFromSymbol(out_host, HIP_SYMBOL(g_dbg_render), sizeof(unsigned) * 4));
  FSN_HIP(hipMemcpyToSymbol(HIP_SYMBOL(g_dbg_render), zero, sizeof(zero)));
  return fsn::debug_report_occ(out_host + 4);
#else
  FSN_REQUIRE(false, FSN_E_UNSUPPORTED, "fsn_debug_report: not a debug build (make -C fs-nerf_amd/csrc debug)");
#endif
}
```

### fs-nerf_amd/csrc/render_occ.hip

```cpp
#include "common.hpp"
#define FSN_KLOOP_ASM
#define FSN_BF16X3_ONEACC 1
#include "mlp_dev.hpp"
#include "occ_dev.hpp"
#include "ray_dev.hpp"

namespace fsn {

FSN_DEBUG_DEFINE_RECORD(g_dbg_occ)
#define FSN_DEBUG_RECORD g_dbg_occ

constexpr int kCap = 2048;
constexpr int kMaxRays = 128;

struct OccKArgs {
  NetParams net;
  fsn_occ_render_args a;
  GridDev G;
  float cam_hw, cam_hh, cam_f;
  int32_t use_vis;
  float cone_angle;
  const float* t_min;
  const float* t_max;
  float* sample_t1;
};

struct OccLds {
  fsn_occ_render_args a;
  GridDev G;
  float cam_hw, cam_hh, cam_f;
  int32_t use_vis;
  float cone_angle;
  const float* t_min;
  const float* t_max;
  float* sample_t1;
  int64_t chunk_base, carry_base;
  int32_t chunk_from, carry_from, chunk_take, carry_take, stop, n_cand, n_kept, n_rays;
  int32_t cnt[kWaves];
  float rays[kMaxRays * 6];
  int64_t ray_id[kMaxRays];
  int32_t cand_off[kMaxRays], cand_cnt[kMaxRays], kept_off[kMaxRays + 1], kept_cnt[kMaxRays];
  float t0c[kCap], sigc[kCap];
  uint16_t slotc[kCap];
  uint8_t keepf[kCap];
  float t0k[kCap], t1k[kCap], rgbk[3 * kCap];
  union {
    float sigk[kCap];
    float t1c[kCap];
  };
  uint16_t slotk[kCap];
};

constexpr int kOccLdsBytes = kRingBytes + (kAuxCapFloats + 96) * 4 + (int)sizeof(OccLds);
static_assert(kOccLdsBytes <= 160 * 1024, "LDS budget");

struct OccSrc {
  const float* ray;
  float t0, t1;
  __device__ __forceinline__ void pos(float& x, float& y, float& z) const {
    const float tm = t0 + t1;
    x = ray[0] + ray[3] * tm / 2.0f;
    y = ray[1] + ray[4] * tm / 2.0f;
    z = ray[2] + ray[5] * tm / 2.0f;
  }
  __device__ __forceinline__ void dir(float& x, float& y, float& z) const { x = ray[3]; y = ray[4]; z = ray[5]; }
};

__device__ __forceinline__ int64_t uniform_i64(int64_t v) {
  const uint32_t lo = (uint32_t)__builtin_amdgcn_readfirstlane((int)(uint32_t)v);
  const uint32_t hi = (uint32_t)__builtin_amdgcn_readfirstlane((int)(uint32_t)((uint64_t)v >> 32));
  return (int64_t)(((uint64_t)hi << 32) | lo);
}

__device__ __forceinline__ int wave_excl_scan_i(int v, int& total) {
  const int lane = lane_id();
  int inc = v;
#pragma unroll
  for (int d = 1; d < 64; d <<= 1) {
    const int o = __shfl_up(inc, d, 64);
    if (lane >= d) inc += o;
  }
  total = __shfl(inc, 63, 64);
  return inc - v;
}

template <int NT, int PREC, bool EX>
__global__ __launch_bounds__(kThreads) void k_render_occ(OccKArgs k) {
  __shared__ __attribute__((aligned(1024))) char smem[kOccLdsBytes];
  float* aux = reinterpret_cast<float*>(smem + kRingBytes);
  OccLds& S = *reinterpret_cast<OccLds*>(smem + kRingBytes + (kAuxCapFloats + 96) * 4);
  int tid = threadIdx.x, wave = tid >> 6, lane = tid & 63;
  if (tid == 0) {
    S.a = k.a; S.G = k.G; S.cam_hw = k.cam_hw; S.cam_hh = k.cam_hh; S.cam_f = k.cam_f; S.use_vis = k.use_vis;
    S.cone_angle = k.cone_angle; S.t_min = k.t_min; S.t_max = k.t_max; S.sample_t1 = k.sample_t1;
    S.carry_from = kWaves; S.carry_base = 0; S.carry_take = 0;
  }
  __syncthreads();
  const fsn_occ_render_args& a = S.a;
  NetDev net;
  load_net(k.net, a.pos_mask, a.dir_mask, aux, net);
  __syncthreads();
  WStream st;
  st.init(smem, nullptr, 0, 0, k.net.blob + k.net.stream_off, WStream::kDynamicPhases, 1);
  const uint32_t nph_density = (uint32_t)k.net.nph_density, nph_full = (uint32_t)k.net.nph_full;
  ARing ring;
  prime_ring<PREC, NT>(st, ring);

  auto cand_end = [&](int i) -> float {
    if constexpr (EX) return FSN_AT(S.t1c, i);
    else return FSN_AT(S.t0c, i) + a.step;
  };
  auto kept_end = [&](int i) -> float {
    if constexpr (EX) return FSN_AT(S.t1k, i);
    else return FSN_AT(S.t0k, i) + a.step;
  };
  auto fetch_ray = [&](int64_t ray, float (&o)[3], float (&d)[3]) {
    if (a.rays_o) {
#pragma unroll
      for (int c = 0; c < 3; ++c) { o[c] = a.rays_o[3 * ray + c]; d[c] = a.rays_d[3 * ray + c]; }
    } else {
      const int h = a.cam_row0 + (int)(ray / a.cam_W), w = (int)(ray % a.cam_W);
      pinhole_ray(a.cam_pose, S.cam_hw, S.cam_hh, S.cam_f, h, w, o, d);
    }
  };

  for (;;) {
    {
      int t_ = threadIdx.x;
      asm volatile("" : "+v"(t_));
      tid = t_; wave = __builtin_amdgcn_readfirstlane(t_ >> 6); lane = t_ & 63;
    }
    if (tid == 0) { S.n_cand = 0; S.n_rays = 0; S.stop = 0; }
    __syncthreads();
    for (;;) {
      if (tid == 0) {
        if (S.carry_from < kWaves) {
          S.chunk_base = S.carry_base; S.chunk_from = S.carry_from; S.chunk_take = S.carry_take; S.carry_from = kWaves;
        } else {
          unsigned long long* wc = reinterpret_cast<unsigned long long*>(a.work_counter);
          const long long seen = (long long)__hip_atomic_load(wc, __ATOMIC_RELAXED, __HIP_MEMORY_SCOPE_AGENT);
          long long take = (a.R - seen) / (2ll * (long long)gridDim.x);
          take = take < 1 ? 1 : (take > kWaves ? kWaves : take);
          S.chunk_base = (int64_t)atomicAdd(wc, (unsigned long long)take);
          S.chunk_from = 0;
          S.chunk_take = (int32_t)take;
        }
      }
      __syncthreads();
      const int64_t base = uniform_i64(S.chunk_base);
      const int from = __builtin_amdgcn_readfirstlane(S.chunk_from), take = __builtin_amdgcn_readfirstlane(S.chunk_take);
      if (base >= a.R) break;
      const int64_t ray = base + wave;
      const bool active = wave >= from && wave < take && ray < a.R;
      float o[3] = {0.f, 0.f, 0.f}, d[3] = {0.f, 0.f, 1.f};
      RayLattice L;
      L.any = false; L.near_r = L.t_lo = L.t_hi = 0.f; L.k0 = 0;
      int c = 0;
      const float cone = EX ? S.cone_angle : 0.f;
      float u_r = 0.f;
      if (active) {
        fetch_ray(ray, o, d);
        u_r = a.u ? a.u[ray] : 0.f;
        if constexpr (EX) {
          const float lo_r = S.t_min ? S.t_min[ray] : -__builtin_huge_valf(), hi_r = S.t_max ? S.t_max[ray] : __builtin_huge_valf();
          L = ray_range(S.G, o, d, a.near_plane, a.far_plane, a.step, cone, a.u != nullptr, u_r, lo_r, hi_r);
          c = march_ray_regime(S.G, a.bits, o, d, L, a.step, cone, a.u != nullptr, u_r, a.max_steps,
                               [](float, float, bool, uint64_t, int) {});
        } else {
          L = ray_lattice(S.G, o, d, a.near_plane, a.far_plane, a.step, a.u != nullptr, u_r);
          c = march_ray(S.G, a.bits, o, d, L, a.step, a.max_steps, [](float, float, bool, uint64_t, int) {});
        }
      }
      if (lane == 0) FSN_AT(S.cnt, wave) = active ? c : -1;
      __syncthreads();
      int nc = S.n_cand, nr = S.n_rays, my_off = -1, my_slot = 0, first_rej = kWaves;
      bool stop = false;
      for (int w = from; w < kWaves; ++w) {
        const int cw = FSN_AT(S.cnt, w);
        if (cw < 0) continue;
        if (!stop && nr < kMaxRays && nc + cw <= kCap) {
          if (w == wave) { my_off = nc; my_slot = nr; }
          nc += cw;
          nr += 1;
        } else if (!stop) {
          stop = true;
          first_rej = w;
        }
      }
      __syncthreads();
      if (tid == 0) {
        S.n_cand = nc; S.n_rays = nr;
        if (stop) { S.carry_base = base; S.carry_from = first_rej; S.carry_take = take; S.stop = 1; }
        else if (take < kWaves) S.stop = 1;
      }
      if (my_off >= 0) {
        if (lane == 0) {
#pragma unroll
          for (int q = 0; q < 3; ++q) { FSN_AT(S.rays, 6 * my_slot + q) = o[q]; FSN_AT(S.rays, 6 * my_slot + 3 + q) = d[q]; }
          FSN_AT(S.ray_id, my_slot) = ray;
          FSN_AT(S.cand_off, my_slot) = my_off;
          FSN_AT(S.cand_cnt, my_slot) = c;
        }
        auto fill = [&](float ts, float te, bool keep, uint64_t m, int before) {
          if (keep) {
            const int pos = my_off + before + __popcll(m & ((1ull << lane) - 1ull));
            FSN_AT(S.t0c, pos) = ts;
            if constexpr (EX) FSN_AT(S.t1c, pos) = te;
            FSN_AT(S.slotc, pos) = (uint16_t)my_slot;
          }
        };
        if constexpr (EX) march_ray_regime(S.G, a.bits, o, d, L, a.step, cone, a.u != nullptr, u_r, a.max_steps, fill);
        else march_ray(S.G, a.bits, o, d, L, a.step, a.max_steps, fill);
      }
      __syncthreads();
      if (S.stop) break;
    }
    const int n_rays = __builtin_amdgcn_readfirstlane(S.n_rays), n_cand = __builtin_amdgcn_readfirstlane(S.n_cand);
    if (n_rays == 0) break;

    constexpr int NG = groups_per_wave<NT, PREC>(), TILE = 128 * NG;
    if (S.use_vis && n_cand > 0) {
      for (int sub = 0; sub * TILE < n_cand; ++sub) {
        const int idx0 = sub * TILE + tile_slot<NG>(wave, lane, 0);
        OccSrc src[NG];
        FSN_PER_GROUP(q, const int ic = min(idx0 + 16 * q, n_cand - 1);
                            src[q] = OccSrc{FSN_SPAN(S.rays, 6 * FSN_AT(S.slotc, ic), 6), FSN_AT(S.t0c, ic), cand_end(ic)};);
        float sigma[NG], rgb[NG][3];
        st.begin_tile(nph_density);
        mlp_tile<NT, PREC, false>(st, net, src, ring, sigma, rgb);
        if (tile_stores<NG>(lane)) {
          const int qs = tile_store_group<NG>(lane), idx = idx0 + 16 * qs;
          if (idx < n_cand) FSN_AT(S.sigc, idx) = sigma[qs];
        }
      }
      lds_barrier();
      for (int r = wave; r < n_rays; r += kWaves) {
        const int Sn = FSN_AT(S.cand_cnt, r), beg = FSN_AT(S.cand_off, r);
        const int per = (Sn + 63) >> 6;
        const int i0 = lane * per, i1 = min(i0 + per, Sn);
        float lsum = 0.f;
        for (int i = i0; i < i1; ++i) lsum += FSN_AT(S.sigc, beg + i) * (cand_end(beg + i) - FSN_AT(S.t0c, beg + i));
        float tot;
        float run = wave_excl_scan(lsum, tot);
        int nk = 0;
        for (int i = i0; i < i1; ++i) {
          const float sdt = FSN_AT(S.sigc, beg + i) * (cand_end(beg + i) - FSN_AT(S.t0c, beg + i));
          const float T = expf(-run), alpha = 1.0f - expf(-sdt);
          const bool kp = T >= a.early_stop_eps && alpha >= a.alpha_thre;
          FSN_AT(S.keepf, beg + i) = kp ? 1 : 0;
          nk += kp ? 1 : 0;
          run += sdt;
        }
        int tk;
// ... 13 lines not shown
      if (2 * lane + 1 < n_rays) FSN_AT(S.kept_off, 2 * lane + 1) = ex + c0;
      if (lane == 0) S.n_kept = tot;
    }
    lds_barrier();
    for (int r = wave; r < n_rays; r += kWaves) {
      const int Sn = FSN_AT(S.cand_cnt, r), beg = FSN_AT(S.cand_off, r), ko = FSN_AT(S.kept_off, r);
      const int per = (Sn + 63) >> 6;
      const int i0 = lane * per, i1 = min(i0 + per, Sn);
      int nk = 0;
      for (int i = i0; i < i1; ++i) nk += FSN_AT(S.keepf, beg + i);
      int tk;
      int pos = ko + wave_excl_scan_i(nk, tk);
      for (int i = i0; i < i1; ++i) {
        if (FSN_AT(S.keepf, beg + i)) {
          FSN_AT(S.t0k, pos) = FSN_AT(S.t0c, beg + i);
          FSN_AT(S.t1k, pos) = cand_end(beg + i);
          FSN_AT(S.slotk, pos) = (uint16_t)r;
          ++pos;
        }
      }
    }
    lds_barrier();
    if (a.sample_t0 && !a.ex_weights) {
      for (int r = wave; r < n_rays; r += kWaves) {
        const int64_t ray = FSN_AT(S.ray_id, r);
        const int ko = FSN_AT(S.kept_off, r), Sk = FSN_AT(S.kept_cnt, r);
        for (int i = lane; i < Sk; i += 64) a.sample_t0[ray * a.sample_cap + i] = FSN_AT(S.t0k, ko + i);
        if constexpr (EX)
          if (S.sample_t1)
            for (int i = lane; i < Sk; i += 64) S.sample_t1[ray * a.sample_cap + i] = FSN_AT(S.t1k, ko + i);
        if (lane == 0) {
          if (a.n_cand) a.n_cand[ray] = FSN_AT(S.cand_cnt, r);
          a.n_kept[ray] = Sk;
        }
      }
      lds_barrier();
      continue;
    }
    const int n_kept = __builtin_amdgcn_readfirstlane(S.n_kept);
    for (int sub = 0; sub * TILE < n_kept; ++sub) {
      const int idx0 = sub * TILE + tile_slot<NG>(wave, lane, 0);
      OccSrc src[NG];
      FSN_PER_GROUP(q, const int ic = min(idx0 + 16 * q, n_kept - 1);
                       src[q] = OccSrc{FSN_SPAN(S.rays, 6 * FSN_AT(S.slotk, ic), 6), FSN_AT(S.t0k, ic), kept_end(ic)};);
      float sigma[NG], rgb[NG][3];
      st.begin_tile(nph_full);
      mlp_tile<NT, PREC, true>(st, net, src, ring, sigma, rgb);
      if (tile_stores<NG>(lane)) {
        const int qs = tile_store_group<NG>(lane), idx = idx0 + 16 * qs;
        if (idx < n_kept) {
          FSN_AT(S.sigk, idx) = sigma[qs];
          FSN_AT(S.rgbk, 3 * idx + 0) = rgb[qs][0];
          FSN_AT(S.rgbk, 3 * idx + 1) = rgb[qs][1];
          FSN_AT(S.rgbk, 3 * idx + 2) = rgb[qs][2];
        }
      }
    }
    lds_barrier();
    for (int r = wave; r < n_rays; r += kWaves) {
      const int64_t ray = FSN_AT(S.ray_id, r);
      const int ko = FSN_AT(S.kept_off, r), Sk = FSN_AT(S.kept_cnt, r);
      const int64_t row = a.ex_weights ? ray * a.sample_cap : 0;
      CompositeOut o{a.colors + 3 * ray, a.opacity + ray, a.depth + ray, a.ex_weights ? a.ex_weights + row : nullptr,
                     a.ex_weights ? a.ex_alphas + row : nullptr, a.ex_weights ? a.ex_trans + row : nullptr};
      composite_ray(FSN_SPAN(S.sigk, ko, Sk), FSN_SPAN(S.rgbk, 3 * ko, 3 * Sk), FSN_SPAN(S.t0k, ko, Sk), FSN_SPAN(S.t1k, ko, Sk), Sk,
                    true, a.bkgd[0], a.bkgd[1], a.bkgd[2], o);
      if (a.ex_weights) {
        for (int i = lane; i < Sk; i += 64) {
          a.sample_t0[row + i] = FSN_AT(S.t0k, ko + i);
          a.ex_sigmas[row + i] = FSN_AT(S.sigk, ko + i);
        }
        if constexpr (EX)
          if (S.sample_t1)
            for (int i = lane; i < Sk; i += 64) S.sample_t1[row + i] = FSN_AT(S.t1k, ko + i);
        for (int i = lane; i < 3 * Sk; i += 64) a.ex_rgbs[3 * row + i] = FSN_AT(S.rgbk, 3 * ko + i);
      }
      if (lane == 0) {
        if (a.n_cand) a.n_cand[ray] = FSN_AT(S.cand_cnt, r);
        if (a.n_kept) a.n_kept[ray] = Sk;
      }
    }
    lds_barrier();
  }
  st.drain();
}

template <int NT, int PREC>
static int launch_occ(const OccKArgs& k, int cus, hipStream_t s) {
  const int64_t chunks = (k.a.R + kWaves - 1) / kWaves;
  const unsigned grid = (unsigned)(chunks < cus ? chunks : cus);
  if (k.cone_angle > 0.f || k.t_min || k.t_max || k.sample_t1) k_render_occ<NT, PREC, true><<<grid, kThreads, 0, s>>>(k);
  else k_render_occ<NT, PREC, false><<<grid, kThreads, 0, s>>>(k);
  FSN_LAUNCH_CHECK("k_render_occ");
  return FSN_OK;
}

}

namespace fsn {
int debug_report_occ(unsigned* host4) {
#ifdef FSN_DEBUG
  unsigned zero[4] = {0u, 0u, 0u, 0u};
  FSN_HIP(hipMemcpyFromSymbol(host4, HIP_SYMBOL(g_dbg_occ), sizeof(unsigned) * 4));
  FSN_HIP(hipMemcpyToSymbol(HIP_SYMBOL(g_dbg_occ), zero, sizeof(zero)));
#else
  for (int i = 0; i < 4; ++i) host4[i] = 0u;
#endif
  return FSN_OK;
}
}

using namespace fsn;

static int occ_render_launch(const char* who, const fsn_mlp_desc* desc, int prec, const void* blob,
                             const fsn_occ_render_args* args, float cone_angle, const float* t_min, const float* t_max,
                             float* sample_t1, fsn_stream_t stream) {
  FSN_REQUIRE(desc && args, FSN_E_INVALID, "%s: null pointer", who);
  const fsn_occ_render_args& a = *args;
  FSN_REQUIRE(a.R >= 0 && a.step > 0.f && a.max_steps > 0, FSN_E_INVALID, "%s: bad sizes", who);
  FSN_REQUIRE(cone_angle >= 0.f, FSN_E_INVALID, "%s: cone_angle must not be negative", who);
  FSN_REQUIRE(!(cone_angle > 0.f && a.near_plane < 0.f), FSN_E_INVALID, "%s: the cone regime needs near_plane >= 0", who);
  FSN_REQUIRE(prec >= 0 && prec <= FSN_PREC_FP16X3U, FSN_E_UNSUPPORTED, "%s: precision mode %d", who, prec);
  NetGeom G;
  const char* why;
  int rc = build_geom(*desc, prec, G, &why);
  FSN_REQUIRE(rc == FSN_OK, rc, "%s: %s", who, why);
  OccKArgs k;
  rc = make_grid(a.aabb, a.res, a.levels, k.G);
  if (rc != FSN_OK) return rc;
  if (a.R == 0) return FSN_OK;
  FSN_REQUIRE(a.rays_o || !(t_min || t_max), FSN_E_INVALID, "%s: per-ray t_min / t_max need ray arrays, not a camera", who);
  FSN_REQUIRE(!(cone_angle > 0.f && a.sample_t0 && !sample_t1), FSN_E_INVALID,
              "%s: the sampler / extras mode in the cone regime needs sample_t1", who);
  FSN_REQUIRE(blob && a.bits && a.work_counter, FSN_E_INVALID, "%s: null pointer", who);
  if (a.ex_weights)
    FSN_REQUIRE(a.sample_t0 && a.ex_alphas && a.ex_trans && a.ex_sigmas && a.ex_rgbs && a.colors && a.opacity && a.depth,
                FSN_E_INVALID, "%s: the extras mode needs sample_t0, all five ex_* arrays and the per-ray outputs", who);
  if (a.sample_t0) {
    FSN_REQUIRE(a.n_kept && a.sample_cap >= a.max_steps, FSN_E_INVALID,
                "%s: the sampler / extras mode needs n_kept and sample_cap >= max_steps", who);
  } else {
    FSN_REQUIRE(a.colors && a.opacity && a.depth, FSN_E_INVALID, "%s: null output pointer", who);
  }
  FSN_REQUIRE(a.max_steps <= kCap, FSN_E_UNSUPPORTED, "%s: max_steps %d > %d samples of one ray group (use the unfused path)",
              who, a.max_steps, kCap);
  if (a.rays_o) {
    FSN_REQUIRE(a.rays_d, FSN_E_INVALID, "%s: rays_o without rays_d", who);
  } else {
    FSN_REQUIRE(a.cam_H > 0 && a.cam_W > 0 && a.cam_focal > 0 && a.cam_row0 >= 0 &&
                    a.R <= (int64_t)(a.cam_H - a.cam_row0) * a.cam_W,
                FSN_E_INVALID, "%s: no rays and no valid camera", who);
  }
  FSN_REQUIRE(G.aux_floats <= kAuxCapFloats, FSN_E_UNSUPPORTED, "%s: network too deep for LDS", who);
  k.net = net_params(*desc, G, blob, a.status);
  k.a = a;
  k.cam_hw = (float)(a.cam_W * 0.5);
  k.cam_hh = (float)(a.cam_H * 0.5);
  k.cam_f = (float)a.cam_focal;
  k.use_vis = (a.early_stop_eps > 0.f || a.alpha_thre > 0.f) ? 1 : 0;
  k.cone_angle = cone_angle;
  k.t_min = t_min;
  k.t_max = t_max;
  k.sample_t1 = a.sample_t0 ? sample_t1 : nullptr;
  const int cus = fsn_device_cus();
  if (cus <= 0) return FSN_E_HIP;
  hipStream_t s = as_stream(stream);
  FSN_HIP(hipMemsetAsync(a.work_counter, 0, sizeof(unsigned long long), s));
  return dispatch_net(PrecModes<FSN_PREC_BF16X3, FSN_PREC_BF16, FSN_PREC_FP16X3, FSN_PREC_FP16, FSN_PREC_FP16X3U>{}, desc->d_hidden,
                      prec, [&](auto NT, auto PREC) { return launch_occ<NT(), PREC()>(k, cus, s); });
}

extern "C" int fsn_render_rays_occgrid(const fsn_mlp_desc* desc, int prec, const void* blob,
                                       const fsn_occ_render_args* args, fsn_stream_t stream) {
  return occ_render_launch("fsn_render_rays_occgrid", desc, prec, blob, args, 0.f, nullptr, nullptr, nullptr, stream);
}

extern "C" int fsn_render_rays_occgrid_ex(const fsn_mlp_desc* desc, int prec, const void* blob,
                                          const fsn_occ_render_args* args, float cone_angle, const float* t_min,
                                          const float* t_max, float* sample_t1, fsn_stream_t stream) {
  return occ_render_launch("fsn_render_rays_occgrid_ex", desc, prec, blob, args, cone_angle, t_min, t_max, sample_t1, stream);
}

namespace fsn {
struct GatherEx {
  const float* slot[5];
  float* out[5];
};
__global__ void k_occ_gather(const int32_t* __restrict__ n_kept, const int64_t* __restrict__ offsets,
                             const float* __restrict__ t0s, const float* __restrict__ t1s, int cap, int64_t R, float step,
                             int64_t* __restrict__ ri, float* __restrict__ ts, float* __restrict__ te, GatherEx ex) {
  const int wave = threadIdx.x >> 6, lane = threadIdx.x & 63;
  const int64_t r = (int64_t)blockIdx.x * 4 + wave;
  if (r >= R) return;
  const int n = n_kept[r];
  const int64_t off = offsets[r];
  for (int i = lane; i < n; i += 64) {
    const float t = t0s[r * cap + i];
    ri[off + i] = r;
    ts[off + i] = t;
    te[off + i] = t1s ? t1s[r * cap + i] : t + step;
  }
  if (ex.slot[0]) {
#pragma unroll
    for (int k = 0; k < 4; ++k)
      for (int i = lane; i < n; i += 64) ex.out[k][off + i] = ex.slot[k][r * cap + i];
    for (int i = lane; i < 3 * n; i += 64) ex.out[4][3 * off + i] = ex.slot[4][3 * r * cap + i];
  }
}
}

static int occ_gather_launch(const char* who, const int32_t* n_kept, const int64_t* offsets, const float* sample_t0,
                             const float* sample_t1, int sample_cap, int64_t R, float step, int64_t* ray_indices,
                             float* t_starts, float* t_ends, bool extras, const float* const* slots, float* const* out,
                             fsn_stream_t stream) {
  FSN_REQUIRE(R >= 0 && sample_cap > 0, FSN_E_INVALID, "%s: bad sizes", who);
  if (R == 0) return FSN_OK;
  FSN_REQUIRE(n_kept && offsets && sample_t0 && ray_indices && t_starts && t_ends && (!extras || (slots && out)),
              FSN_E_INVALID, "%s: null pointer", who);
  GatherEx ex{};
  if (extras)
    for (int k = 0; k < 5; ++k) {
      FSN_REQUIRE(slots[k] && out[k], FSN_E_INVALID, "%s: null slot / output array %d", who, k);
      ex.slot[k] = slots[k];
      ex.out[k] = out[k];
    }
  k_occ_gather<<<(unsigned)((R + 3) / 4), 256, 0, as_stream(stream)>>>(n_kept, offsets, sample_t0, sample_t1, sample_cap, R,
                                                                       step, ray_indices, t_starts, t_ends, ex);
  FSN_LAUNCH_CHECK("k_occ_gather");
  return FSN_OK;
}

extern "C" int fsn_occ_gather_samples(const int32_t* n_kept, const int64_t* offsets, const float* sample_t0, int sample_cap,
                                      int64_t R, float step, int64_t* ray_indices, float* t_starts, float* t_ends,
                                      fsn_stream_t stream) {
  return occ_gather_launch("fsn_occ_gather_samples", n_kept, offsets, sample_t0, nullptr, sample_cap, R, step, ray_indices,
                           t_starts, t_ends, false, nullptr, nullptr, stream);
}

extern "C" int fsn_occ_gather_extras(const int32_t* n_kept, const int64_t* offsets, const float* sample_t0, int sample_cap,
                                     int64_t R, float step, int64_t* ray_indices, float* t_starts, float* t_ends,
                                     const float* const* slots, float* const* out, fsn_stream_t stream) {
  return occ_gather_launch("fsn_occ_gather_extras", n_kept, offsets, sample_t0, nullptr, sample_cap, R, step, ray_indices,
                           t_starts, t_ends, true, slots, out, stream);
}

extern "C" int fsn_occ_gather_ex(const int32_t* n_kept, const int64_t* offsets, const float* sample_t0,
                                 const float* sample_t1, int sample_cap, int64_t R, float step, int64_t* ray_indices,
                                 float* t_starts, float* t_ends, const float* const* slots, float* const* out,
                                 fsn_stream_t stream) {
  FSN_REQUIRE(!slots == !out, FSN_E_INVALID, "fsn_occ_gather_ex: slots and outputs come together");
  return occ_gather_launch("fsn_occ_gather_ex", n_kept, offsets, sample_t0, sample_t1, sample_cap, R, step, ray_indices,
                           t_starts, t_ends, slots != nullptr, slots, out, stream);
}
```

### fs-nerf_amd/csrc/train_fused.hip

```cpp
#define FSN_X3_PF1
#include <type_traits>

#include "mlp_dev.hpp"
#include "mlp_layout.hpp"
#include "train_internal.hpp"

namespace fsn {

typedef __attribute__((ext_vector_type(16))) float f32x16;
typedef __attribute__((ext_vector_type(2))) float f32x2;

constexpr int kTC = kTileCols;

struct FusedLayout {
  int L, D, NT, d_pe, d_de, prec;
  int64_t T;
  int64_t blob_f, blob_b;
  int64_t pe, de, h, h_stride, bo, dhead, dbo, dp, part, hpart, total;
  int64_t mask, mask_stride;
  int nsplit[4], nsplit_heads, n_bwd_units, nph_bwd;
  int64_t blob_f_bytes;
};

enum { WG_BIG = 0, WG_ENC = 1, WG_BR = 2, WG_BD = 3 };
// ... 841 lines not shown
  };
  for (int64_t t = t0; t < t1; ++t) {
    const float* dht = a.dhead + t * 4 * kTC;
    if (wave == 0) {
#pragma unroll
      for (int c = 0; c < 4; ++c) {
        const f32x2 d2 = *reinterpret_cast<const f32x2*>(dht + c * kTC + 2 * lane);
        accB[c] += d2[0] + d2[1];
      }
    }
    const uint32_t* hp = a.H + t * D * kTC + ((PH * wave + qh) * kTRow + s4) * NPL;
#pragma unroll
    for (int c0 = 0; c0 < NCH; c0 += CH) {
      const int c = c0 + ch;
      const f32x4 ds = *reinterpret_cast<const f32x4*>(dht + 3 * kTC + 16 * c + s4);
      float h[2][4];
      load_pair(hp + (int64_t)c * (D / 2) * kTRow * NPL, h);
#pragma unroll
      for (int i = 0; i < 4; ++i) {
        accS[0] += ds[i] * h[0][i];
        accS[1] += ds[i] * h[1][i];
      }
    }
    const uint32_t* bp = a.Bo + t * (D / 2) * kTC + ((PB * wave + qb) * kTRow + s4) * NPL;
#pragma unroll
    for (int c0 = 0; c0 < NCH; c0 += CB) {
      const int c = c0 + cb;
      float b[2][4];
      load_pair(bp + (int64_t)c * (D / 4) * kTRow * NPL, b);
#pragma unroll
      for (int k = 0; k < 3; ++k) {
        const f32x4 dz = *reinterpret_cast<const f32x4*>(dht + k * kTC + 16 * c + s4);
#pragma unroll
        for (int i = 0; i < 4; ++i) {
          accR[k][0] += dz[i] * b[0][i];
          accR[k][1] += dz[i] * b[1][i];
        }
      }
    }
  }
  float* out = a.hpart + (int64_t)blockIdx.x * (D + 3 * (D / 2) + 4);
  auto rsum = [&](float v, int P) {
    v += __shfl_xor(v, 1, 64);
    v += __shfl_xor(v, 2, 64);
    for (int mm = 4 * P; mm < 64; mm <<= 1) v += __shfl_xor(v, mm, 64);
    return v;
  };
#pragma unroll
  for (int par = 0; par < 2; ++par) {
    const float v = rsum(accS[par], PH);
    if ((lane & 3) == 0 && ch == 0) out[2 * PH * wave + 2 * qh + par] = v;
  }
#pragma unroll
  for (int k = 0; k < 3; ++k)
#pragma unroll
    for (int par = 0; par < 2; ++par) {
      const float v = rsum(accR[k][par], PB);
      if ((lane & 3) == 0 && cb == 0) out[D + k * (D / 2) + 2 * PB * wave + 2 * qb + par] = v;
    }
  if (wave == 0) {
#pragma unroll
    for (int c = 0; c < 4; ++c) {
      float v = accB[c];
#pragma unroll
      for (int mm = 32; mm >= 1; mm >>= 1) v += __shfl_xor(v, mm, 64);
      if (lane == 0) out[D + 3 * (D / 2) + c] = v;
    }
  }
}

struct HeadsRdArgs {
  const float* hpart;
  int32_t nsplit, D;
  const float* scale;
  float *dWs, *dbs, *dWr, *dbr;
  const uint32_t* status;
  int32_t accumulate;
};
__global__ void k_heads_reduce(HeadsRdArgs a) {
  const int e = blockIdx.x * blockDim.x + threadIdx.x;
  const int n = a.D + 3 * (a.D / 2) + 4;
  if (e >= n) return;
  const float inv = a.scale ? 1.0f / a.scale[0] : 1.0f;
  float sum = sum_partials(a.hpart + e, n, a.nsplit) * inv;
  if (a.status && (a.status[0] & (FSN_STATUS_FP16_RANGE | FSN_STATUS_GRAD_RANGE))) sum = 0.f;
  float* dst;
  if (e < a.D) dst = a.dWs + e;
  else if (e < a.D + 3 * (a.D / 2)) dst = a.dWr + (e - a.D);
  else if (e < n - 1) dst = a.dbr + (e - a.D - 3 * (a.D / 2));
  else dst = a.dbs;
  *dst = a.accumulate ? *dst + sum : sum;
}

__global__ void k_bwd_rescale(float* __restrict__ bs, uint32_t* __restrict__ amax, int n) {
  const int i = threadIdx.x;
  if (i >= n) return;
  const uint32_t m = amax[i];
  amax[i] = 0u;
  if (m == 0u) return;
  float f = bs[i];
  if (m >= 0x7c00u) {
    f *= 0.00390625f;
  } else {
    const int e = (m >> 10) ? (int)(m >> 10) - 15 : (31 - __builtin_clz(m)) - 24;
    f = ldexpf(f, 5 - e);
  }
  bs[i] = fminf(fmaxf(f, 5.9604644775390625e-08f), 1.099511627776e12f);
}

int64_t fused_train_workspace_floats(const fsn_mlp_desc& d, int prec, int64_t n) {
  FusedLayout F;
  const char* why;
  const int rc = make_fused_layout(d, prec, n, F, &why);
  FSN_REQUIRE(rc == FSN_OK, rc, "training path: %s", why);
  return F.total;
}

template <int NT, int PREC>
static int launch_fwd(const TrainFwdArgs& a, unsigned grid, hipStream_t s) {
  k_train_fwd<NT, PREC><<<grid, kThreads, 0, s>>>(a);
  FSN_LAUNCH_CHECK("k_train_fwd");
  return FSN_OK;
}
template <int NT, int PREC>
static int launch_bwd(const TrainBwdArgs& a, unsigned grid, hipStream_t s) {
  k_train_bwd<NT, PREC><<<grid, kThreads, 0, s>>>(a);
  FSN_LAUNCH_CHECK("k_train_bwd");
  return FSN_OK;
}
template <int NW, int MG, int BT>
static int launch_wgrad(int prec, const WgArgs& a, int njobs, hipStream_t s) {
  if (njobs == 0) return FSN_OK;
  const int a_rows = a.job[0].a_rows;
  FSN_REQUIRE(a_rows % (64 * MG) == 0, FSN_E_HIP, "internal: wgrad row blocks");
  dim3 grid((unsigned)a.nsplit, (unsigned)njobs, (unsigned)(a_rows / (64 * MG)));
  return dispatch_prec(PrecTraining{}, prec, [&](auto PREC) {
    k_wgrad<NW, MG, BT, PREC()><<<grid, 64 * NW, 0, s>>>(a);
    FSN_LAUNCH_CHECK("k_wgrad");
    return FSN_OK;
  });
}

int fused_train_fwd(const fsn_mlp_desc* d, int prec, const float* const* W, const float* const* b, const float* x,
                    const float* dirs, const float* pos_mask, const float* dir_mask, int64_t n, float* ws, float* out,
                    uint32_t* status, hipStream_t s, const TrainRays* rays) {
  FusedLayout F;
  const char* why;
  int rc = make_fused_layout(*d, prec, n, F, &why);
  FSN_REQUIRE(rc == FSN_OK, rc, "fsn_nerf_train_fwd: %s", why);
  NetGeom G;
  build_geom(*d, prec, G, &why);
  FSN_REQUIRE(G.aux_floats <= kAuxCapFloats, FSN_E_UNSUPPORTED, "fsn_nerf_train_fwd: network too deep for the LDS aux area");
  void* blob = ws + F.blob_f;
  rc = fsn_mlp_pack(d, prec, W, b, blob, (fsn_stream_t)s);
  if (rc != FSN_OK) return rc;
  const int cus = fsn_device_cus();
  if (cus <= 0) return FSN_E_HIP;
  TrainFwdArgs a{net_params(*d, G, blob, status), x, dirs, pos_mask, dir_mask, n, out, ws, F.h, F.h_stride, F.bo, F.pe, F.de,
                 F.mask, F.mask_stride, F.D, nullptr, nullptr, nullptr, nullptr, nullptr};
  if (rays) { a.rays_o = rays->rays_o; a.rays_d = rays->rays_d; a.t0 = rays->t0; a.t1 = rays->t1; a.ri = rays->ri; }
  const unsigned grid = (unsigned)(F.T < cus ? F.T : cus);
  return dispatch_net(PrecTraining{}, F.D, prec, [&](auto NT, auto PREC) { return launch_fwd<NT(), PREC()>(a, grid, s); });
}

int fused_train_bwd(const fsn_mlp_desc* d, int prec, const float* const* W, int64_t n, float* ws, const float* out,
                    const float* d_out, const float* grad_scale_dev, float* const* dW, float* const* db,
                    bool accumulate, float* bscale, uint32_t* bamax, uint32_t* status, hipStream_t s,
                    const InputGradReq* ig) {
  FusedLayout F;
  const char* why;
  int rc = make_fused_layout(*d, prec, n, F, &why);
  FSN_REQUIRE(rc == FSN_OK, rc, "fsn_nerf_train_bwd: %s", why);
  NetGeom G;
  build_geom(*d, prec, G, &why);
  const int cus = fsn_device_cus();
  if (cus <= 0) return FSN_E_HIP;
  const int L = F.L, D = F.D, NT = F.NT;
  {
    BwdPackArgs p{};
    int u = 0, gi = 0;
    p.W[gi] = W[L + 2]; p.ld[gi] = D + F.d_de; p.ks[gi] = NT / 2; p.unit0[gi] = u; u += 2 * NT * (NT / 2); ++gi;
    p.W[gi] = W[L + 1]; p.ld[gi] = D; p.ks[gi] = NT; p.unit0[gi] = u; u += 2 * NT * NT; ++gi;
    for (int l = L - 1; l >= 1; --l) {
      const bool wide = (d->skip_mask >> (l - 1)) & 1u;
      p.W[gi] = W[l]; p.ld[gi] = D + (wide ? F.d_pe : 0); p.ks[gi] = NT; p.unit0[gi] = u; u += 2 * NT * NT; ++gi;
    }
    p.n_gemm = gi; p.units_total = u; p.prec = prec; p.NT = NT;
    FSN_REQUIRE(u == F.n_bwd_units, FSN_E_HIP, "internal: backward unit count");
    const int64_t n_pieces = (int64_t)F.nph_bwd * kPhaseBytes / 16;
    k_pack_bwd<<<(unsigned)((n_pieces + 255) / 256), 256, 0, s>>>(p, reinterpret_cast<char*>(ws + F.blob_b), n_pieces);
    FSN_LAUNCH_CHECK("k_pack_bwd");
  }
  {
    TrainBwdArgs a{net_params(*d, G, ws + F.blob_f, status), reinterpret_cast<const char*>(ws + F.blob_b), F.nph_bwd, n, out, d_out,
                   grad_scale_dev, ws, F.h, F.h_stride, F.bo, F.dhead, F.dbo, F.dp, F.mask, F.mask_stride,
                   prec_is_f16(prec) ? bscale : nullptr, prec_is_f16(prec) ? bamax : nullptr};
    const unsigned grid = (unsigned)(F.T < cus ? F.T : cus);
    rc = dispatch_net(PrecTraining{}, D, prec, [&](auto NT, auto PREC) { return launch_bwd<NT(), PREC()>(a, grid, s); });
    if (rc != FSN_OK) return rc;
  }
  auto rescale = [&]() {
    if (prec_is_f16(prec) && bscale && bamax) {
      k_bwd_rescale<<<1, 64, 0, s>>>(bscale, bamax, L + 2);
      FSN_LAUNCH_CHECK("k_bwd_rescale");
    }
    return FSN_OK;
  };
  if (ig) {
    const InputGradWs o{F.blob_b, F.pe - F.blob_b, F.dp, F.h_stride, F.dbo};
    rc = input_grad_launch(*d, prec, W, n, ws, o, grad_scale_dev, prec_is_f16(prec) ? bscale : nullptr,
                           prec_is_f16(prec) ? status : nullptr, *ig, s);
    if (rc != FSN_OK) return rc;
  }
  if (!dW) return rescale();
  WgArgs wa[4] = {};
  int cnt[4] = {0, 0, 0, 0};
  RdArgs rd{};
  int nrd = 0;
  float* part = ws + F.part;
  auto U = [](const float* q) { return reinterpret_cast<const uint32_t*>(q); };
  auto H = [&](int i) { return ws + F.h + i * F.h_stride; };
  auto dP = [&](int i) { return ws + F.dp + i * F.h_stride; };
  auto add = [&](int kind, int stage, const float* A, const float* B, int a_rows, int b_rows, bool bias, float* dWp, float* dbp,
                 int ld, int col0, int mode, int n_freqs) {
    const int64_t ns = F.nsplit[kind];
    WgJob& j = wa[kind].job[cnt[kind]++];
    j.A = U(A); j.B = U(B); j.b_rows = b_rows; j.a_rows = a_rows;
    j.part = part; part += ns * a_rows * b_rows;
    j.bpart = nullptr;
    if (bias) { j.bpart = part; part += ns * a_rows; }
    RdJob& r = rd.job[nrd++];
    r.part = j.part; r.bpart = j.bpart; r.dW = dWp; r.db = dbp; r.a_rows = a_rows; r.b_rows = b_rows; r.ld = ld;
    r.col0 = col0; r.mode = mode; r.n_freqs = n_freqs; r.nsplit = (int)ns; r.stage = stage;
  };
  for (int l = 1; l < L; ++l) {
    const bool wide = (d->skip_mask >> (l - 1)) & 1u;
    add(WG_BIG, l, dP(l), H(l - 1), D, D, true, dW[l], db[l], D + (wide ? F.d_pe : 0), 0, 0, 0);
    if (wide) add(WG_ENC, l, dP(l), ws + F.pe, D, 64, false, dW[l], nullptr, D + F.d_pe, D, 1, d->n_freqs_pos);
  }
  add(WG_BIG, L, dP(L), H(L - 1), D, D, true, dW[L + 1], db[L + 1], D, 0, 0, 0);
  add(WG_ENC, 0, dP(0), ws + F.pe, D, 64, true, dW[0], db[0], F.d_pe, 0, 1, d->n_freqs_pos);
  add(WG_BR, L + 1, ws + F.dbo, H(L), D / 2, D, true, dW[L + 2], db[L + 2], D + F.d_de, 0, 0, 0);
  add(WG_BD, L + 1, ws + F.dbo, ws + F.de, D / 2, 32, false, dW[L + 2], nullptr, D + F.d_de, D, 2, d->n_freqs_dir);
  FSN_REQUIRE(part - (ws + F.part) <= part_floats(*d, F.nsplit), FSN_E_HIP, "internal: wgrad partial area");
  for (int k = 0; k < 4; ++k) { wa[k].T = F.T; wa[k].nsplit = F.nsplit[k]; }
  const WgArgs &big = wa[WG_BIG], &enc = wa[WG_ENC], &br = wa[WG_BR], &bd = wa[WG_BD];
  const int nbig = cnt[WG_BIG], nenc = cnt[WG_ENC], nbr = cnt[WG_BR], nbd = cnt[WG_BD];
  if (D == 256) {
    if ((rc = launch_wgrad<8, 4, 4>(prec, big, nbig, s)) != FSN_OK) return rc;
    if ((rc = launch_wgrad<8, 4, 1>(prec, enc, nenc, s)) != FSN_OK) return rc;
    if ((rc = launch_wgrad<8, 2, 2>(prec, br, nbr, s)) != FSN_OK) return rc;
    if ((rc = launch_wgrad<8, 2, 1>(prec, bd, nbd, s)) != FSN_OK) return rc;
  } else {
    if ((rc = launch_wgrad<8, 2, 1>(prec, big, nbig, s)) != FSN_OK) return rc;
    if ((rc = launch_wgrad<8, 2, 1>(prec, enc, nenc, s)) != FSN_OK) return rc;
    if ((rc = launch_wgrad<8, 1, 1>(prec, br, nbr, s)) != FSN_OK) return rc;
    if ((rc = launch_wgrad<8, 1, 1>(prec, bd, nbd, s)) != FSN_OK) return rc;
  }
  rd.scale = grad_scale_dev;
  rd.status = prec_is_f16(prec) ? status : nullptr;
  rd.accumulate = accumulate ? 1 : 0;
  rd.bscale = prec_is_f16(prec) ? bscale : nullptr;
  {
    dim3 grid((unsigned)((D * D + 255) / 256), (unsigned)nrd);
    k_wgrad_reduce<<<grid, 256, 0, s>>>(rd);
    FSN_LAUNCH_CHECK("k_wgrad_reduce");
  }
  {
    HeadsArgs ha{U(H(L - 1)), U(ws + F.bo), ws + F.dhead, ws + F.hpart, F.T, F.nsplit_heads};
    const unsigned hg = (unsigned)F.nsplit_heads;
    rc = dispatch_net(PrecTraining{}, D, prec, [&](auto NT, auto PREC) {
      k_heads_wgrad<NT(), PREC()><<<hg, kThreads, 0, s>>>(ha);
      FSN_LAUNCH_CHECK("k_heads_wgrad");
      return FSN_OK;
    });
    if (rc != FSN_OK) return rc;
    HeadsRdArgs hr{ws + F.hpart, F.nsplit_heads, D, grad_scale_dev, dW[L], db[L], dW[L + 3], db[L + 3],
                   prec_is_f16(prec) ? status : nullptr, accumulate ? 1 : 0};
    const int nn = D + 3 * (D / 2) + 4;
    k_heads_reduce<<<(unsigned)((nn + 255) / 256), 256, 0, s>>>(hr);
    FSN_LAUNCH_CHECK("k_heads_reduce");
  }
  return rescale();
}

}
```

### fs-nerf_amd/csrc/train_internal.hpp

```cpp
#pragma once
#include "common.hpp"

namespace fsn {

struct TrainRays {
  const float *rays_o, *rays_d, *t0, *t1;
  const int64_t* ri;
};

struct InputGradReq {
  const float *x, *dirs;
  const TrainRays* rays;
  const float *pos_mask, *dir_mask;
  float *d_x, *d_dirs;
};

int64_t fused_train_workspace_floats(const fsn_mlp_desc& d, int prec, int64_t n);
int fused_train_fwd(const fsn_mlp_desc* d, int prec, const float* const* W, const float* const* b, const float* x,
                    const float* dirs, const float* pos_mask, const float* dir_mask, int64_t n, float* ws, float* out,
                    uint32_t* status, hipStream_t s, const TrainRays* rays = nullptr);
int fused_train_bwd(const fsn_mlp_desc* d, int prec, const float* const* W, int64_t n, float* ws, const float* out,
                    const float* d_out, const float* grad_scale_dev, float* const* dW, float* const* db,
                    bool accumulate, float* bscale, uint32_t* bamax, uint32_t* status, hipStream_t s,
                    const InputGradReq* ig = nullptr);

int check_desc(const fsn_mlp_desc* d);
int train_bwd_checked(const char* who, const fsn_mlp_desc* desc, int prec, const float* const* W, int64_t n, float* ws,
                      const float* out, const float* d_out, const float* grad_scale, float* const* dW, float* const* db,
                      int accumulate, float* stage_scales, uint32_t* stage_amax, uint32_t* status, fsn_stream_t stream,
                      const InputGradReq* rq);

struct InputGradWs {
  int64_t blob, blob_floats;
  int64_t dp, h_stride, dbo;
};
int input_grad_launch(const fsn_mlp_desc& d, int prec, const float* const* W, int64_t n, float* ws, const InputGradWs& o,
                      const float* grad_scale_dev, const float* bscale, const uint32_t* status, const InputGradReq& rq,
                      hipStream_t s);

}
```

Baseline: 1.631 million.

## Fold connection layer into RGB branch weights for inference full pass

Precomputes the product of the branch and connection weights (and the folded bias) at pack time, and stores a second weight stream in the blob that uses the fused matrix. In inference and render full passes the connection GEMM is skipped and the branch reads the last hidden activations directly. This removes one 256x256 layer per fine sample. The cost is a larger blob, extra pack work, and a calibration adjustment so the folded weights stay within fp16 range. Accuracy may shift slightly because the folded weights are rounded once in a different place.

```diff
diff --git a/fs-nerf_amd/core/models.py b/fs-nerf_amd/core/models.py
--- a/fs-nerf_amd/core/models.py
+++ b/fs-nerf_amd/core/models.py
@@ -331,6 +331,7 @@
             na = 0 if g == 0 else D
             wmax.append(w[:, :na].amax() if na else w.new_zeros(()))
             wmax.append(w[:, na:].amax() if w.shape[1] > na else w.new_zeros(()))
+        wmax.append((self.branch.weight.detach()[:, :D] @ self.connection.weight.detach()).abs().amax())
         host = torch.cat([maxima, torch.stack(wmax).to(torch.float32)]).cpu().tolist()
         amax, wmx = host[:n + 2], host[n + 2:]
         T = int(self.act_target_exp)
@@ -353,6 +354,11 @@
                     over = math.ceil(math.log2(wm)) + sh - 15
                     if over > 0:
                         exps[g] -= over
+        wm = wmx[2 * (n + 2)]
+        if wm > 0.0 and math.isfinite(wm):
+            over = math.ceil(math.log2(wm)) + exps[n + 1] - exps[n - 1] - 15
+            if over > 0:
+                exps[n + 1] -= over
         self._act_exps = exps
         self._calib_key = self._param_key()
         self._needs_calibration = False
diff --git a/fs-nerf_amd/csrc/host_pack.cpp b/fs-nerf_amd/csrc/host_pack.cpp
--- a/fs-nerf_amd/csrc/host_pack.cpp
+++ b/fs-nerf_amd/csrc/host_pack.cpp
@@ -20,7 +20,7 @@
   const char* why;
   const int rc = fsn::build_geom(*desc, prec, G, &why);
   if (rc != FSN_OK) { set_error("fsn_mlp_blob_bytes: %s", why); return rc; }
-  return G.total_bytes;
+  return G.blob_bytes;
 }
 
 extern "C" int fsn_mlp_pack_host(const fsn_mlp_desc* desc, int prec, const float* const* weights,
diff --git a/fs-nerf_amd/csrc/mlp.hip b/fs-nerf_amd/csrc/mlp.hip
--- a/fs-nerf_amd/csrc/mlp.hip
+++ b/fs-nerf_amd/csrc/mlp.hip
@@ -1,29 +1,48 @@
 #include "common.hpp"
 #define FSN_X3_PF1
 #define FSN_BF16X3_ONEACC 1
+#define FSN_FOLD_FULL_PASS 1
 #include "mlp_dev.hpp"
 #include "mlp_layout.hpp"
 #include "mlp_pack.hpp"
+#include "train_internal.hpp"
 
 #include <cstring>
 #include <vector>
 
 namespace fsn {
 
-__global__ void k_pack_stream(PackArgs a, char* __restrict__ blob, int64_t n_pieces) {
-  const int64_t piece = (int64_t)blockIdx.x * blockDim.x + threadIdx.x;
-  if (piece >= n_pieces) return;
+__global__ void k_pack_stream(PackArgs a, char* __restrict__ blob, int64_t n_pieces, int64_t n_hidden) {
+  int64_t piece = (int64_t)blockIdx.x * blockDim.x + threadIdx.x;
   uint16_t o[8];
-  pack_piece(a, piece, o);
+  int64_t dst, dst2 = 0;
+  if (piece < n_pieces) {
+    pack_piece(a, piece, o);
+    dst = a.G.stream_off + piece * 16;
+    if (piece < n_hidden) dst2 = a.G.fold_stream_off + piece * 16;
+  } else {
+    piece = piece - n_pieces + n_hidden;
+    if (!a.with_fold || piece >= (int64_t)a.G.fold_nph * (kPhaseBytes / 16)) return;
+    pack_fold_piece(a, piece, reinterpret_cast<const float*>(blob + a.G.fold_w_off), o);
+    dst = a.G.fold_stream_off + piece * 16;
+  }
   uint4 v;
   v.x = o[0] | ((uint32_t)o[1] << 16);
   v.y = o[2] | ((uint32_t)o[3] << 16);
   v.z = o[4] | ((uint32_t)o[5] << 16);
   v.w = o[6] | ((uint32_t)o[7] << 16);
-  *reinterpret_cast<uint4*>(blob + a.G.stream_off + piece * 16) = v;
-}
-
-__global__ void k_pack_aux(PackArgs a, char* __restrict__ blob) {
+  *reinterpret_cast<uint4*>(blob + dst) = v;
+  if (dst2) *reinterpret_cast<uint4*>(blob + dst2) = v;
+}
+
+__global__ void k_pack_aux(PackArgs a, char* __restrict__ blob, int aux_blocks) {
+  if ((int)blockIdx.x >= aux_blocks) {
+    const int D = a.d_hidden;
+    const int f = ((int)blockIdx.x - aux_blocks) * blockDim.x + threadIdx.x;
+    if (f < (D / 2) * D) reinterpret_cast<float*>(blob + a.G.fold_w_off)[f] = fold_weight(a, f / D, f % D);
+    else if (f < (D / 2) * D + D) reinterpret_cast<float*>(blob + a.G.fold_bias_off)[f - (D / 2) * D] = fold_bias(a, f - (D / 2) * D);
+    return;
+  }
   const int i = blockIdx.x * blockDim.x + threadIdx.x;
   if (i < 64) {
     uint32_t hw[64];
@@ -37,9 +56,9 @@
 }
 
 static int fill_pack_args(const fsn_mlp_desc* d, int prec, const float* const* W, const float* const* b,
-                          PackArgs& a, const int32_t* exps = nullptr) {
-  const char* why;
-  const int rc = fill_pack_args_raw(d, prec, W, b, a, &why, exps);
+                          PackArgs& a, const int32_t* exps, bool with_fold) {
+  const char* why;
+  const int rc = fill_pack_args_raw(d, prec, W, b, a, &why, exps, with_fold);
   FSN_REQUIRE(rc == FSN_OK, rc, "mlp_pack: %s", why);
   return FSN_OK;
 }
@@ -64,7 +83,7 @@
   float* aux_lds = reinterpret_cast<float*>(smem + kRingBytes);
   float* in_lds = aux_lds + kAuxCapFloats + 96;
   NetDev net;
-  load_net(a.net, a.pos_mask, a.dir_mask, aux_lds, net);
+  load_net<(FULL && tile_folds(PREC)) ? 32 * NT : 0>(a.net, a.pos_mask, a.dir_mask, aux_lds, net);
   __syncthreads();
   constexpr bool full = FULL;
   const int64_t ntiles = (a.n + TILE - 1) / TILE;
@@ -203,7 +222,7 @@
   const char* why;
   const int rc = build_geom(*desc, prec, G, &why);
   FSN_REQUIRE(rc == FSN_OK, rc, "fsn_mlp_blob_bytes: %s", why);
-  return G.total_bytes;
+  return G.blob_bytes;
 }
 
 extern "C" int fsn_mlp_pack(const fsn_mlp_desc* desc, int prec, const float* const* weights, const float* const* biases,
@@ -211,19 +230,31 @@
   return fsn_mlp_pack_scaled(desc, prec, weights, biases, nullptr, blob, stream);
 }
 
+namespace fsn {
+int mlp_pack_device(const fsn_mlp_desc* desc, int prec, const float* const* weights, const float* const* biases,
+                    const int32_t* layer_exps, void* blob, bool with_fold, hipStream_t stream) {
+  FSN_REQUIRE(blob, FSN_E_INVALID, "fsn_mlp_pack: null blob");
+  PackArgs a;
+  const int rc = fill_pack_args(desc, prec, weights, biases, a, layer_exps, with_fold);
+  if (rc != FSN_OK) return rc;
+  const bool fold = with_fold && a.G.fold_nph > 0;
+  const int D = a.d_hidden;
+  const int naux = a.G.aux_floats > 64 ? a.G.aux_floats : 64;
+  const int aux_blocks = (naux + 255) / 256, fold_blocks = fold ? ((D / 2) * D + D + 255) / 256 : 0;
+  k_pack_aux<<<(unsigned)(aux_blocks + fold_blocks), 256, 0, stream>>>(a, static_cast<char*>(blob), aux_blocks);
+  FSN_LAUNCH_CHECK("k_pack_aux");
+  const int64_t n_pieces = (int64_t)a.G.nph_full * kPhaseBytes / 16;
+  const int64_t n_hidden = fold ? (int64_t)a.G.nph_density * kPhaseBytes / 16 : 0;
+  const int64_t n_tail = fold ? (int64_t)a.G.fold_nph * kPhaseBytes / 16 - n_hidden : 0;
+  k_pack_stream<<<(unsigned)((n_pieces + n_tail + 255) / 256), 256, 0, stream>>>(a, static_cast<char*>(blob), n_pieces, n_hidden);
+  FSN_LAUNCH_CHECK("k_pack_stream");
+  return FSN_OK;
+}
+}
+
 extern "C" int fsn_mlp_pack_scaled(const fsn_mlp_desc* desc, int prec, const float* const* weights,
                                    const float* const* biases, const int32_t* layer_exps, void* blob, fsn_stream_t stream) {
-  FSN_REQUIRE(blob, FSN_E_INVALID, "fsn_mlp_pack: null blob");
-  PackArgs a;
-  const int rc = fill_pack_args(desc, prec, weights, biases, a, layer_exps);
-  if (rc != FSN_OK) return rc;
-  const int64_t n_pieces = (int64_t)a.G.nph_full * kPhaseBytes / 16;
-  k_pack_stream<<<(unsigned)((n_pieces + 255) / 256), 256, 0, as_stream(stream)>>>(a, static_cast<char*>(blob), n_pieces);
-  FSN_LAUNCH_CHECK("k_pack_stream");
-  const int naux = a.G.aux_floats > 64 ? a.G.aux_floats : 64;
-  k_pack_aux<<<(unsigned)((naux + 255) / 256), 256, 0, as_stream(stream)>>>(a, static_cast<char*>(blob));
-  FSN_LAUNCH_CHECK("k_pack_aux");
-  return FSN_OK;
+  return mlp_pack_device(desc, prec, weights, biases, layer_exps, blob, true, as_stream(stream));
 }
 
 extern "C" int fsn_mlp_pack_host(const fsn_mlp_desc* desc, int prec, const float* const* weights,
@@ -256,7 +287,7 @@
   FSN_REQUIRE(G.aux_floats <= kAuxCapFloats, FSN_E_UNSUPPORTED, "%s: network too deep for the LDS aux area", who);
   const int cus = fsn_device_cus();
   if (cus <= 0) return FSN_E_HIP;
-  a.net = net_params(*desc, G, blob, status);
+  a.net = net_params(*desc, G, blob, status, tile_folds(prec) && (a.dirs || (a.ri && a.full)));
   hipStream_t s = as_stream(stream);
   return dispatch_net(PrecInference{}, desc->d_hidden, prec, [&](auto NT, auto PREC) { return launch_mlp_fwd<NT(), PREC()>(a, cus, s); });
 }
diff --git a/fs-nerf_amd/csrc/mlp_dev.hpp b/fs-nerf_amd/csrc/mlp_dev.hpp
--- a/fs-nerf_amd/csrc/mlp_dev.hpp
+++ b/fs-nerf_amd/csrc/mlp_dev.hpp
@@ -55,6 +55,10 @@
 #ifndef FSN_BF16X3_ONEACC
 #define FSN_BF16X3_ONEACC 0
 #endif
+#ifndef FSN_FOLD_FULL_PASS
+#define FSN_FOLD_FULL_PASS 0
+#endif
+constexpr bool tile_folds(int prec) { return FSN_FOLD_FULL_PASS && prec_folds(prec); }
 constexpr bool prec_one_acc(int P) { return P == FSN_PREC_FP16X3U || (FSN_BF16X3_ONEACC && P == FSN_PREC_BF16X3); }
 
 struct Frag {
@@ -294,16 +298,23 @@
   int32_t n_layers;
   uint32_t skip_mask;
   int32_t n_freqs_pos, n_freqs_dir;
+  int32_t fold_bias_off;
   uint32_t* status;
 };
 
-inline NetParams net_params(const fsn_mlp_desc& d, const NetGeom& G, const void* blob, uint32_t* status) {
+inline NetParams net_params(const fsn_mlp_desc& d, const NetGeom& G, const void* blob, uint32_t* status, bool fold = false) {
   NetParams p;
   p.blob = static_cast<const char*>(blob);
   p.aux_off = (int32_t)G.aux_off; p.aux_floats = G.aux_floats; p.stream_off = (int32_t)G.stream_off;
   p.nph_density = G.nph_density; p.nph_full = G.nph_full;
   p.n_layers = d.n_layers; p.skip_mask = d.skip_mask;
   p.n_freqs_pos = d.n_freqs_pos; p.n_freqs_dir = d.n_freqs_dir;
+  p.fold_bias_off = 0;
+  if (fold) {
+    p.stream_off = (int32_t)G.fold_stream_off;
+    p.nph_full = G.fold_nph;
+    p.fold_bias_off = (int32_t)G.fold_bias_off;
+  }
   p.status = status;
   return p;
 }
@@ -968,8 +979,9 @@
     FSN_PER_GROUP(q, sg[q] += __shfl_xor(sg[q], 32, 64););
     FSN_PER_GROUP(q, sigma[q] = sg[q] + misc[0];);
   }
+  constexpr bool FOLD = FULL && tile_folds(PREC) && std::is_same<SV, NoSave>::value;
   if (FULL) {
-    {
+    if constexpr (!FOLD) {
       typename SV::Hook hk = sv.hidden(L);
       FSN_GEMM_LAYER((PREC, NT, NA, 0, EPI_CVT), L * D, B, none, A);
       sv.layer_done(L, hk);
@@ -979,7 +991,8 @@
                   encode<kKsDir, F16, X3, SV::kSave, LS>(dx, dy, dz, net.n_freqs_dir, misc + 20, net.dir_mask, g, de[q], sv.enc_dir(g)););
     {
       typename SV::Hook hk = sv.branch();
-      FSN_GEMM_LAYER((PREC, NT / 2, NA, kKsDir, EPI_RGB), (L + 1) * D, A, de, B);
+      if constexpr (FOLD) FSN_GEMM_LAYER((PREC, NT / 2, NA, kKsDir, EPI_RGB), (L + 1) * D, B, de, A);
+      else FSN_GEMM_LAYER((PREC, NT / 2, NA, kKsDir, EPI_RGB), (L + 1) * D, A, de, B);
       sv.layer_done(L + 1, hk);
     }
 #pragma unroll
@@ -1026,11 +1039,18 @@
   }
 }
 
+template <int FOLD_D = 0>
 __device__ __forceinline__ void load_net(const NetParams& p, const float* __restrict__ pos_mask_g,
                                          const float* __restrict__ dir_mask_g, float* lds, NetDev& net) {
   const f32x4* src = reinterpret_cast<const f32x4*>(p.blob + p.aux_off);
   f32x4* dst = reinterpret_cast<f32x4*>(lds);
-  for (int i = threadIdx.x; i < p.aux_floats / 4; i += blockDim.x) dst[i] = src[i];
+  if constexpr (FOLD_D != 0) {
+    const f32x4* fb = reinterpret_cast<const f32x4*>(p.blob + p.fold_bias_off);
+    const int b0 = (p.n_layers + 1) * (FOLD_D / 4);
+    for (int i = threadIdx.x; i < p.aux_floats / 4; i += blockDim.x) dst[i] = (i >= b0 && i < b0 + FOLD_D / 4) ? fb[i - b0] : src[i];
+  } else {
+    for (int i = threadIdx.x; i < p.aux_floats / 4; i += blockDim.x) dst[i] = src[i];
+  }
   float* pm = lds + p.aux_floats;
   float* dm = pm + 64;
   const int npe = 3 * (1 + 2 * p.n_freqs_pos), nde = 3 * (1 + 2 * p.n_freqs_dir);
diff --git a/fs-nerf_amd/csrc/mlp_layout.hpp b/fs-nerf_amd/csrc/mlp_layout.hpp
--- a/fs-nerf_amd/csrc/mlp_layout.hpp
+++ b/fs-nerf_amd/csrc/mlp_layout.hpp
@@ -24,6 +24,7 @@
 constexpr float kLoScaleF16 = 2048.0f;
 FSN_HD constexpr bool prec_lo_scaled(int prec) { return prec == FSN_PREC_FP16X3 || prec == FSN_PREC_FP16X2; }
 FSN_HD float lo_scale(int prec) { return prec_lo_scaled(prec) ? kLoScaleF16 : 1.0f; }
+FSN_HD constexpr bool prec_folds(int prec) { return prec_reads_w_lo(prec); }
 FSN_HD int unit_bytes(int prec) { return prec_is_x3(prec) ? 2048 : 1024; }
 FSN_HD int units_per_phase(int prec) { return kPhaseBytes / unit_bytes(prec); }
 
@@ -47,6 +48,10 @@
   int32_t aux_bias[kMaxLayers + 2];
   int32_t aux_wsigma, aux_wrgb, aux_misc, aux_floats;
   int64_t aux_off, stream_off, total_bytes;
+  LayerGeom fold_branch;
+  int32_t fold_units, fold_nph;
+  int64_t fold_bias_off, fold_w_off, fold_stream_off;
+  int64_t blob_bytes;
 };
 
 FSN_HD int enc_slot_feature(int q, int g, int n_freqs, int slots) {
@@ -161,6 +166,19 @@
   G.aux_off = 256;
   G.stream_off = (G.aux_off + (int64_t)G.aux_floats * 4 + 4095) / 4096 * 4096;
   G.total_bytes = G.stream_off + (int64_t)G.nph_full * kPhaseBytes;
+  G.fold_branch = b;
+  G.fold_branch.unit0 = G.units_hidden;
+  G.fold_units = G.fold_nph = 0;
+  G.fold_bias_off = G.fold_w_off = G.fold_stream_off = 0;
+  G.blob_bytes = G.total_bytes;
+  if (prec_is_x3(prec)) {
+    G.fold_units = G.units_hidden + 2 * b.nt_out * (b.ks_act + b.ks_enc);
+    G.fold_nph = (G.fold_units + upp - 1) / upp;
+    G.fold_bias_off = G.total_bytes;
+    G.fold_w_off = G.fold_bias_off + (int64_t)D * 4;
+    G.fold_stream_off = (G.fold_w_off + (int64_t)(D / 2) * D * 4 + 4095) / 4096 * 4096;
+    G.blob_bytes = G.fold_stream_off + (int64_t)G.fold_nph * kPhaseBytes;
+  }
   return FSN_OK;
 }
 
diff --git a/fs-nerf_amd/csrc/mlp_pack.hpp b/fs-nerf_amd/csrc/mlp_pack.hpp
--- a/fs-nerf_amd/csrc/mlp_pack.hpp
+++ b/fs-nerf_amd/csrc/mlp_pack.hpp
@@ -13,6 +13,8 @@
   float freqs_pos[16], freqs_dir[16];
   int32_t exps[kMaxLayers + 2];
   float sc_act[kMaxLayers + 2], sc_enc[kMaxLayers + 2], sc_bias[kMaxLayers + 2], sc_sigma, sc_rgb;
+  int32_t with_fold;
+  float sc_fold;
 };
 
 FSN_HD float pow2f(int e) {
@@ -33,9 +35,16 @@
   }
   a.sc_sigma = pow2f(-a.exps[L - 1]);
   a.sc_rgb = pow2f(-a.exps[L + 1]);
+  a.sc_fold = pow2f(a.exps[L + 1] - a.exps[L - 1]);
 }
 
 FSN_HD int gemm_to_sd(int g, int L) { return g < L ? g : g + 1; }
+
+FSN_HD uint16_t weight_part(float w, int part, int prec) {
+  const bool f16 = prec_is_f16(prec);
+  const uint16_t hi = half_rne(w, f16);
+  return part == 0 ? hi : half_rne((w - half_to_f32(hi, f16)) * lo_scale(prec), f16);
+}
 
 FSN_HD void pack_piece(const PackArgs& a, int64_t piece, uint16_t out8[8]) {
   const int ub = unit_bytes(a.prec);
@@ -59,9 +68,50 @@
     const int col = unit_src_col(Lg, ks, grp, j);
     if (col < 0) continue;
     const float w = W[(int64_t)row * Lg.ld + col] * (ks < Lg.ks_act ? a.sc_act[g] : a.sc_enc[g]);
-    const bool f16 = prec_is_f16(a.prec);
-    const uint16_t hi = half_rne(w, f16);
-    out8[j] = part == 0 ? hi : half_rne((w - half_to_f32(hi, f16)) * lo_scale(a.prec), f16);
+    out8[j] = weight_part(w, part, a.prec);
+  }
+}
+
+FSN_HD float fold_weight(const PackArgs& a, int o, int k) {
+  const int D = a.d_hidden, L = a.n_layers;
+  const float* Wc = a.W[L + 1] + k;
+  const float* Wb = a.W[L + 2] + (int64_t)o * a.G.fold_branch.ld;
+  double s = 0.0;
+#pragma unroll 16
+  for (int j = 0; j < D; ++j) s = __builtin_fma((double)Wb[j], (double)Wc[(int64_t)j * D], s);
+  return (float)s * a.sc_fold;
+}
+FSN_HD float fold_bias(const PackArgs& a, int o) {
+  const int D = a.d_hidden, L = a.n_layers;
+  if (o >= D / 2) return 0.f;
+  const float* Wb = a.W[L + 2] + (int64_t)o * a.G.fold_branch.ld;
+  const float* bc = a.b[L + 1];
+  double s = 0.0;
+#pragma unroll 16
+  for (int j = 0; j < D; ++j) s = __builtin_fma((double)Wb[j], (double)bc[j], s);
+  return (float)(s + (double)a.b[L + 2][o]) * a.sc_bias[L + 1];
+}
+FSN_HD void pack_fold_piece(const PackArgs& a, int64_t piece, const float* wf, uint16_t out8[8]) {
+  const int ppu = unit_bytes(a.prec) / 16;
+  const int unit = (int)(piece / ppu);
+  const int rem = (int)(piece - (int64_t)unit * ppu);
+  const int part = rem >> 6, lane = rem & 63;
+  for (int j = 0; j < 8; ++j) out8[j] = 0;
+  if (unit < a.G.units_hidden || unit >= a.G.fold_units) return;
+  const LayerGeom& Lg = a.G.fold_branch;
+  const int g = a.n_layers + 1;
+  const int ks_tot = Lg.ks_act + Lg.ks_enc;
+  const int lu = unit - Lg.unit0;
+  const int sub = lu & 1;
+  const int t = (lu >> 1) / ks_tot, ks = (lu >> 1) - t * ks_tot;
+  const int r = lane & 15, grp = lane >> 4;
+  const float* Wb = a.W[gemm_to_sd(g, a.n_layers)];
+  const int row = 32 * t + 16 * sub + r;
+  for (int j = 0; j < 8; ++j) {
+    const int col = unit_src_col(Lg, ks, grp, j);
+    if (col < 0) continue;
+    const float w = ks < Lg.ks_act ? wf[(int64_t)row * a.d_hidden + col] : Wb[(int64_t)row * Lg.ld + col] * a.sc_enc[g];
+    out8[j] = weight_part(w, part, a.prec);
   }
 }
 
@@ -93,11 +143,16 @@
   hw[7] = (uint32_t)a.n_freqs_dir; hw[8] = (uint32_t)a.G.units_total; hw[9] = (uint32_t)a.G.nph_full;
   hw[10] = (uint32_t)a.G.nph_density; hw[11] = (uint32_t)a.G.aux_off; hw[12] = (uint32_t)a.G.aux_floats;
   hw[13] = (uint32_t)a.G.stream_off; hw[14] = (uint32_t)(a.G.total_bytes & 0xffffffffu);
+  if (a.with_fold && a.G.fold_nph) {
+    hw[36] = (uint32_t)a.G.fold_stream_off; hw[37] = (uint32_t)a.G.fold_nph; hw[38] = (uint32_t)a.G.fold_units;
+    hw[39] = (uint32_t)a.G.fold_bias_off; hw[40] = (uint32_t)a.G.fold_w_off;
+    hw[41] = (uint32_t)(a.G.blob_bytes & 0xffffffffu);
+  }
 }
 
 
 inline int fill_pack_args_raw(const fsn_mlp_desc* d, int prec, const float* const* W, const float* const* b, PackArgs& a,
-                              const char** why, const int32_t* exps = nullptr) {
+                              const char** why, const int32_t* exps = nullptr, bool with_fold = true) {
   *why = "";
   if (!d || !W || !b) { *why = "null pointer"; return FSN_E_INVALID; }
   const int rc = build_geom(*d, prec, a.G, why);
@@ -114,6 +169,7 @@
     for (int g = 0; g < d->n_layers + 2; ++g)
       if (exps[g] < -60 || exps[g] > 60) { *why = "layer exponent outside [-60, 60]"; return FSN_E_INVALID; }
   fill_scales(a, exps);
+  a.with_fold = with_fold ? 1 : 0;
   return FSN_OK;
 }
 
@@ -123,7 +179,7 @@
   const int rc = fill_pack_args_raw(d, prec, W, b, a, why, exps);
   if (rc != FSN_OK) return rc;
   char* blob = static_cast<char*>(blob_host);
-  for (int64_t i = 0; i < a.G.total_bytes; ++i) blob[i] = 0;
+  for (int64_t i = 0; i < a.G.blob_bytes; ++i) blob[i] = 0;
   uint32_t hw[64];
   header_words(a, hw);
   for (int i = 0; i < 64; ++i) reinterpret_cast<uint32_t*>(blob)[i] = hw[i];
@@ -132,6 +188,18 @@
   const int64_t n_pieces = (int64_t)a.G.nph_full * kPhaseBytes / 16;
   uint16_t* sp = reinterpret_cast<uint16_t*>(blob + a.G.stream_off);
   for (int64_t p = 0; p < n_pieces; ++p) pack_piece(a, p, sp + p * 8);
+  if (a.with_fold && a.G.fold_nph) {
+    float* fb = reinterpret_cast<float*>(blob + a.G.fold_bias_off);
+    float* wf = reinterpret_cast<float*>(blob + a.G.fold_w_off);
+    const int D = a.d_hidden;
+    for (int o = 0; o < D; ++o) fb[o] = fold_bias(a, o);
+    for (int o = 0; o < D / 2; ++o)
+      for (int k = 0; k < D; ++k) wf[(int64_t)o * D + k] = fold_weight(a, o, k);
+    uint16_t* fs = reinterpret_cast<uint16_t*>(blob + a.G.fold_stream_off);
+    const int64_t n_hidden = (int64_t)a.G.nph_density * kPhaseBytes / 16, n_fold = (int64_t)a.G.fold_nph * kPhaseBytes / 16;
+    for (int64_t i = 0; i < n_hidden * 8; ++i) fs[i] = sp[i];
+    for (int64_t p = n_hidden; p < n_fold; ++p) pack_fold_piece(a, p, wf, fs + p * 8);
+  }
   return FSN_OK;
 }
 
diff --git a/fs-nerf_amd/csrc/render.hip b/fs-nerf_amd/csrc/render.hip
--- a/fs-nerf_amd/csrc/render.hip
+++ b/fs-nerf_amd/csrc/render.hip
@@ -91,7 +91,7 @@
   }
   __syncthreads();
   NetDev netC, netF;
-  load_net(k.netF, a.pos_mask, a.dir_mask, auxF, netF);
+  load_net<tile_folds(PREC) ? 32 * NT : 0>(k.netF, a.pos_mask, a.dir_mask, auxF, netF);
   if (GRP_HIER) load_net(k.netC, a.pos_mask, a.dir_mask, auxC, netC);
   else netC = netF;
   __syncthreads();
@@ -399,7 +399,7 @@
   }
   FSN_REQUIRE(G.aux_floats <= kAuxCapFloats, FSN_E_UNSUPPORTED, "fsn_render_rays_fused: network too deep for LDS");
   RenderKArgs k;
-  k.netF = net_params(*desc, G, blob_fine, a.status);
+  k.netF = net_params(*desc, G, blob_fine, a.status, tile_folds(prec));
   k.netC = net_params(*desc, G, a.n_imp > 0 ? blob_coarse : blob_fine, a.status);
   k.a = a;
   k.G = k.nsubC = k.nsubF = 0;
diff --git a/fs-nerf_amd/csrc/render_occ.hip b/fs-nerf_amd/csrc/render_occ.hip
--- a/fs-nerf_amd/csrc/render_occ.hip
+++ b/fs-nerf_amd/csrc/render_occ.hip
@@ -1,6 +1,7 @@
 #include "common.hpp"
 #define FSN_KLOOP_ASM
 #define FSN_BF16X3_ONEACC 1
+#define FSN_FOLD_FULL_PASS 1
 #include "mlp_dev.hpp"
 #include "occ_dev.hpp"
 #include "ray_dev.hpp"
@@ -98,7 +99,7 @@
   __syncthreads();
   const fsn_occ_render_args& a = S.a;
   NetDev net;
-  load_net(k.net, a.pos_mask, a.dir_mask, aux, net);
+  load_net<tile_folds(PREC) ? 32 * NT : 0>(k.net, a.pos_mask, a.dir_mask, aux, net);
   __syncthreads();
   WStream st;
   st.init(smem, nullptr, 0, 0, k.net.blob + k.net.stream_off, WStream::kDynamicPhases, 1);
@@ -418,7 +419,7 @@
                 FSN_E_INVALID, "%s: no rays and no valid camera", who);
   }
   FSN_REQUIRE(G.aux_floats <= kAuxCapFloats, FSN_E_UNSUPPORTED, "%s: network too deep for LDS", who);
-  k.net = net_params(*desc, G, blob, a.status);
+  k.net = net_params(*desc, G, blob, a.status, tile_folds(prec));
   k.a = a;
   k.cam_hw = (float)(a.cam_W * 0.5);
   k.cam_hh = (float)(a.cam_H * 0.5);
diff --git a/fs-nerf_amd/csrc/train_fused.hip b/fs-nerf_amd/csrc/train_fused.hip
--- a/fs-nerf_amd/csrc/train_fused.hip
+++ b/fs-nerf_amd/csrc/train_fused.hip
@@ -1017,7 +1017,7 @@
   build_geom(*d, prec, G, &why);
   FSN_REQUIRE(G.aux_floats <= kAuxCapFloats, FSN_E_UNSUPPORTED, "fsn_nerf_train_fwd: network too deep for the LDS aux area");
   void* blob = ws + F.blob_f;
-  rc = fsn_mlp_pack(d, prec, W, b, blob, (fsn_stream_t)s);
+  rc = mlp_pack_device(d, prec, W, b, nullptr, blob, false, s);
   if (rc != FSN_OK) return rc;
   const int cus = fsn_device_cus();
   if (cus <= 0) return FSN_E_HIP;
diff --git a/fs-nerf_amd/csrc/train_internal.hpp b/fs-nerf_amd/csrc/train_internal.hpp
--- a/fs-nerf_amd/csrc/train_internal.hpp
+++ b/fs-nerf_amd/csrc/train_internal.hpp
@@ -24,6 +24,9 @@
                     bool accumulate, float* bscale, uint32_t* bamax, uint32_t* status, hipStream_t s,
                     const InputGradReq* ig = nullptr);
 
+int mlp_pack_device(const fsn_mlp_desc* desc, int prec, const float* const* weights, const float* const* biases,
+                    const int32_t* layer_exps, void* blob, bool with_fold, hipStream_t stream);
+
 int check_desc(const fsn_mlp_desc* d);
 int train_bwd_checked(const char* who, const fsn_mlp_desc* desc, int prec, const float* const* W, int64_t n, float* ws,
                       const float* out, const float* d_out, const float* grad_scale, float* const* dW, float* const* db,
```

Result: no change. 1.625 million (-0.4%).
